# xxxupeng/stereo_toolbox

Hardware: AMD Instinct MI355X
Metric: stereo pairs/sec @ 540x960 D=192 (GwcNet_GC fwd+bwd) (higher is better)
Workload: dtype f32; 1 GPU; GwcNet_GC(maxdisp=192) train step: fwd+bwd+allreduce+Adam, 576x960 pairs (reference pad_to_2x shape), batch 1/GPU, fp32, synthetic randn inputs, deterministic filler weights; global_batch=1, parallelism=dp1, grad_sync=none (single rank: flat fp32 buffer packed, no collective), launch=eager, optimizer=torch.optim.Adam(fused=True)

## Files before the change

include/stx_hip.h:

```cpp
#ifndef STX_HIP_H
#define STX_HIP_H
#ifdef __cplusplus
extern "C" {
#endif

const char* stx_last_error(void);
const char* stx_build_info(void);
int stx_get_tuning(const char* name);
int stx_set_tuning(const char* name, int value);

int stx_cost_volume_fwd(const float* Lg, const float* Rg, int Cg, int G, const float* Lc, const float* Rc, int Cc,
                        const float* scale, float* vol, int B, int H, int W, int D, int mask_left, void* stream);
int stx_group_normalize_fwd(const float* x, float* y, int B, int C, int G, int HW, float out_scale, void* stream);
int stx_group_normalize_bwd(const float* x, const float* gy, float* gx, int B, int C, int G, int HW, float out_scale, void* stream);
int stx_cost_volume_bwd(const float* gvol, const float* Lg, const float* Rg, int Cg, int G, int Cc, float* gLg,
                        float* gRg, float* gLc, float* gRc, int B, int H, int W, int D, int mask_left, void* stream);

int stx_head_fwd(const float* cost, float* disp, float* stats, int B, int Dc, int Hc, int Wc, int D, int H, int W,
                 void* stream);
long long stx_head_bwd_workspace_floats(int B, int Dc, int H, int W);
int stx_head_bwd(const float* gdisp, const float* cost, const float* disp, const float* stats, float* gcost,
                 float* workspace, int B, int Dc, int Hc, int Wc, int D, int H, int W, void* stream);
int stx_head_fwd2(const float* cost, float* disp, float* stats, int B, int Dc, int Hc, int Wc, int D, int H, int W,
                  int align_corners, void* stream);
int stx_head_bwd2(const float* gdisp, const float* cost, const float* disp, const float* stats, float* gcost,
                  float* workspace, int B, int Dc, int Hc, int Wc, int D, int H, int W, int align_corners, void* stream);
int stx_softargmax_fwd(const float* x, float* out, int B, int D, int HW, void* stream);
int stx_argmax_fwd(const float* x, long long* out, int B, int D, int HW, void* stream);
int stx_unimodal_fwd(const float* x, float* out, int B, int D, int HW, void* stream);
int stx_dominant_modal_fwd(const float* x, float* out, int B, int D, int HW, void* stream);
int stx_modal_fwd(const float* x, float* out, float* aux, int B, int D, int HW, int kind, void* stream);
int stx_modal_bwd(const float* g, const float* out, const float* aux, float* gx, int B, int D, int HW, void* stream);
int stx_split_mode(const float* x, float* mode, unsigned char* mask, int B, int D, int HW, void* stream);
int stx_softmax_d_fwd(const float* x, float* y, int B, int D, int HW, void* stream);

long long stx_conv3d_packed_floats(int K, int N, int T);
int stx_conv3d_pack_weight(const float* w, float* wp, int A, int B, int T, int mode, void* stream);
int stx_conv3d_fwd_blocks(int Do, int Ho, int Wo);
long long stx_conv3d_fwd_stat_rows(int B, int Di, int Hi, int Wi, int Cin, int Cout, int ks, int stride);
int stx_conv3d_fwd(const float* x, const float* wp, float* out, const float* scale, const float* bias,
                   const float* residual, float* stats, int B, int Di, int Hi, int Wi, int Cin, int Cout, int ks,
                   int stride, int relu, void* stream);
int stx_deconv3d_fwd_blocks(int Di, int Hi, int Wi);
int stx_deconv3d_fwd(const float* x, const float* wp, float* out, const float* scale, const float* bias,
                     const float* residual, float* stats, int B, int Di, int Hi, int Wi, int Cin, int Cout, int Do,
                     int Ho, int Wo, int relu, void* stream);
long long stx_conv3d_wgrad_workspace_floats(int B, int Dc, int Hc, int Wc, int CF, int CC, int ks, int stride);
int stx_conv3d_wgrad(const float* fine, const float* coarse, float* dw, float* workspace, int B, int Df, int Hf, int Wf,
                     int CF, int Dc, int Hc, int Wc, int CC, int ks, int stride, void* stream);

int stx_conv3d_wgrad_bn_supported(int B, int D, int H, int W, int CF, int CC);
int stx_conv3d_wgrad_bn(const float* x, const float* gy, const float* z, const float* scale, const float* shift, const float* mean,
                        const float* invstd, const float* gamma, const float* sums, float inv_n, int act, float* dz, float* dw,
                        float* workspace, int B, int D, int H, int W, int CF, int CC, void* stream);

int stx_conv2d_supported(int Cin, int Cout);
long long stx_conv2d_stat_rows(int groups);
int stx_conv2d_fwd(const float* x, const float* w, float* out, float* stats, int B, int H, int W, int Cin, int Cout, int dgrad,
                   int groups, void* stream);

int stx_conv3d_c1_fwd(const float* x, const float* w, const float* residual, float* out, int B, int D, int H, int W,
                      int Cin, void* stream);
long long stx_conv3d_c1_wgrad_workspace_floats(int Cin);
int stx_conv3d_c1_wgrad(const float* x, const float* gy, float* dw, float* workspace, int B, int D, int H, int W,
                        int Cin, void* stream);
int stx_conv3d_c1_dgrad(const float* gy, const float* w, float* gx, int B, int D, int H, int W, int Cin, void* stream);

int stx_mish_fwd(const float* x, float* y, long long n, void* stream);
int stx_mish_bwd(const float* gy, const float* x, float* gx, long long n, void* stream);
int stx_depth_to_space(const float* y, float* out, int B, int D, int H, int W, int C, int inverse, void* stream);
int stx_gate_fwd(const float* cv, const float* att, float* out, int B, int D, long long HW, int C, void* stream);
int stx_gate_bwd(const float* g, const float* cv, const float* att, float* gcv, float* gatt, int B, int D, long long HW,
                 int C, void* stream);

int stx_concat_channels(const float* in0, const float* in1, const float* in2, const float* in3, int C0, int C1, int C2, int C3,
                        float* out, long long nvox, void* stream);
int stx_split_channels(const float* in, float* out0, float* out1, float* out2, float* out3, int C0, int C1, int C2, int C3,
                       long long nvox, void* stream);
int stx_transpose(const float* in, float* out, int N, int rows, int cols, void* stream);

int stx_dwconv_hw_fwd(const float* x, const float* w, const int* dil, float* out, int B, int D, int H, int W, int C,
                      int flip, void* stream);
long long stx_dwconv_hw_wgrad_workspace_floats(int C);
int stx_dwconv_hw_wgrad(const float* x, const float* gy, const int* dil, float* dw, float* workspace, int B, int D,
                        int H, int W, int C, void* stream);
int stx_cost_volume_scale_bwd(const float* gvol, const float* Lc, const float* Rc, float* gscale, int B, int Cc, int H,
                              int W, int D, int mask_left, void* stream);
int stx_scale_channels(const float* x, const float* s, float* out, long long nvox, int C, void* stream);
int stx_ac_volume_bwd(const float* gvol, const float* Lc, const float* Rc, const float* prob, float* gL, float* gR,
                      float* gprob, int B, int Cc, int H, int W, int D, int mask_left, void* stream);

int stx_bn_reduce_blocks(void);
int stx_bn_stats_rows(long long nvox, int C);
int stx_bn_stats(const float* z, float* partials, long long nvox, int C, int groups, void* stream);
int stx_bn_finalize(const float* partials, int nrows, int C, double count, const float* gamma, const float* beta,
                    float* running_mean, float* running_var, float momentum, float eps, float* scale, float* shift,
                    float* mean, float* invstd, void* stream);
int stx_bn_finalize_groups(const float* partials, int nrows, int C, double count, const float* gamma, const float* beta,
                           float* running_mean, float* running_var, float momentum, float eps, float* out, int groups,
                           void* stream);
int stx_bn_apply(const float* z1, const float* scale1, const float* shift1, const float* z2, const float* scale2,
                 const float* shift2, float* out, long long nvox, int C, int relu, int groups, void* stream);
int stx_bn_bwd_reduce(const float* gy, const float* y, const float* z1, const float* mean1, const float* invstd1,
                      const float* z2, const float* mean2, const float* invstd2, float* partials, float* sums,
                      long long nvox, int C, int relu, void* stream);
int stx_bn_bwd_apply(const float* gy, const float* y, const float* z1, const float* mean1, const float* invstd1,
                     const float* gamma1, const float* z2, const float* mean2, const float* invstd2,
                     const float* gamma2, const float* sums, float* dz1, float* dz2, float* gout, long long nvox, int C,
                     int relu, void* stream);
int stx_bn_bwd_reduce2(const float* gy, const float* y, const float* z1, const float* mean1, const float* invstd1,
                       const float* z2, const float* mean2, const float* invstd2, const float* scale1,
                       const float* shift1, const float* scale2, const float* shift2, float* partials, float* sums,
                       long long nvox, int C, int relu, int groups, void* stream);
int stx_bn_bwd_apply2(const float* gy, const float* y, const float* z1, const float* mean1, const float* invstd1,
                      const float* gamma1, const float* z2, const float* mean2, const float* invstd2,
                      const float* gamma2, const float* scale1, const float* shift1, const float* scale2,
                      const float* shift2, const float* sums, float* dz1, float* dz2, float* gout, long long nvox,
                      int C, int relu, int groups, void* stream);

int stx_pad_normalize_u8(const unsigned char* img, float* out, int B, int H, int W, int Hp, int Wp, int top,
                         const float* mean3, const float* std3, void* stream);

int stx_sampled_volume_fwd(const float* Lg, const float* Rg, int Cg, int G, const float* Lc, const float* Rc, int Cc,
                           const float* samples, float* vol, int B, int H, int W, int S, int CTp, void* stream);
int stx_sampled_volume_bwd(const float* gvol, const float* Lg, const float* Rg, int Cg, int G, int Cc,
                           const float* samples, float* gLg, float* gRg, float* gLc, float* gRc, int B, int H, int W,
                           int S, int CTp, void* stream);

int stx_warp_fwd(const float* x, const float* disp, float* out, int B, int C, int H, int W, void* stream);
int stx_warp_bwd(const float* gout, const float* x, const float* disp, float* gx, float* gdisp, int B, int C, int H, int W,
                 void* stream);
int stx_corr_volume_fwd(const float* ref, const float* tgt, float* vol, int B, int C, int H, int W, int maxdisp, int groups,
                        void* stream);
int stx_corr_volume_bwd(const float* gvol, const float* ref, const float* tgt, float* gref, float* gtgt, int B, int C, int H,
                        int W, int maxdisp, int groups, void* stream);
int stx_disparity_variance_fwd(const float* x, const float* disp, const float* samples, float* out, int B, int D, int HW,
                               void* stream);
int stx_disparity_variance_bwd(const float* g, const float* x, const float* disp, const float* samples, float* gx, float* gdisp,
                               float* gsamples, int B, int D, int HW, void* stream);

long long stx_geo_pyramid_floats(long long rows, int len, int C, int levels);
int stx_geo_corr_fwd(const float* fmap1, const float* fmap2, float* cpyr, int B, int C, int H, int W1, int W2, int levels,
                     void* stream);
int stx_geo_corr_bwd(const float* gcpyr, const float* fmap1, const float* fmap2, float* gfmap1, float* gfmap2, int B, int C, int H,
                     int W1, int W2, int levels, void* stream);
int stx_geo_pyramid_fwd(const float* vol, float* gpyr, int B, int D, int H, int W, int C, int levels, void* stream);
int stx_geo_pyramid_bwd(const float* ggpyr, float* gvol, int B, int D, int H, int W, int C, int levels, void* stream);
int stx_geo_lookup_fwd(const float* gpyr, const float* cpyr, const float* disp, const float* coords, float* out, int B, int H,
                       int W, int D, int C, int W2, int levels, int radius, void* stream);
int stx_geo_lookup_bwd(const float* gout, const float* disp, const float* coords, float* ggpyr, float* gcpyr, int B, int H, int W,
                       int D, int C, int W2, int levels, int radius, void* stream);
int stx_context_upsample_fwd(const float* disp_low, const float* up_weights, float* out, int B, int h, int w, void* stream);
int stx_context_upsample_bwd(const float* g, const float* disp_low, const float* up_weights, float* gdisp, float* gweights, int B,
                             int h, int w, void* stream);

long long stx_corr1d_pyramid_floats(long long rows, int W2, int levels);
int stx_corr1d_pyramid_fwd(const float* fmap1, const float* fmap2, float* cpyr, int B, int C, int H, int W1, int W2, int levels,
                           float scale, void* stream);
int stx_corr1d_pyramid_bwd(const float* gcpyr, const float* fmap1, const float* fmap2, float* gfmap1, float* gfmap2, int B, int C,
                           int H, int W1, int W2, int levels, float scale, void* stream);
int stx_corr1d_lookup_fwd(const float* cpyr, const float* base, const float* disp, const float* jobs, int njobs, float* out, int B,
                          int H, int W1, int W2, int levels, void* stream);
int stx_corr1d_lookup_bwd(const float* gout, const float* base, const float* disp, const float* jobs, int njobs, float* gcpyr,
                          int B, int H, int W1, int W2, int levels, void* stream);

int stx_allpairs_estimates_fwd(const float* vol, int which, float* disp_l, float* conf_l, float* disp_r, float* conf_r, float* stats,
                               int B, int H, int W1, int W2, void* stream);
int stx_allpairs_estimates_bwd(const float* g_disp_l, const float* g_conf_l, const float* g_disp_r, const float* g_conf_r,
                               const float* vol, const float* stats, float* gvol, int B, int H, int W1, int W2, void* stream);
int stx_corr1d_volume_pyramid_fwd(const float* vol, const float* tdisp, const float* tconf, float atten, float* cpyr, int B, int H,
                                  int W1, int W2, int levels, void* stream);
int stx_corr1d_volume_pyramid_bwd(const float* gcpyr, const float* tdisp, const float* tconf, float atten, float* gvol, int B, int H,
                                  int W1, int W2, int levels, void* stream);
int stx_truncate_mask_fwd(const float* disp, const float* conf, int has_th, float conf_th, float atten, float* mask, int B, int H,
                          int W, void* stream);

int stx_photo_warp_fwd(const float* right, const float* disp, float* warped, float* valid, int B, int C, int H, int W, void* stream);
int stx_photo_warp_bwd(const float* gwarped, const float* right, const float* disp, float* gdisp, int B, int C, int H, int W,
                       void* stream);
int stx_ssim_fwd(const float* x, const float* y, float* out, int B, int C, int H, int W, int window, void* stream);
long long stx_ssim_bwd_workspace_floats(int B, int C, int H, int W);
int stx_ssim_bwd(const float* g_out, const float* x, const float* y, float* gx, float* gy, float* workspace, int B, int C, int H, int W,
                 int window, void* stream);
int stx_photometric_fwd(const float* left, const float* right, const float* disp, double ssim_weight, int enable_mask, float* loss,
                        int B, int C, int H, int W, void* stream);
long long stx_photometric_bwd_workspace_floats(int B, int C, int H, int W);
int stx_photometric_bwd(const float* gloss, const float* left, const float* right, const float* disp, double ssim_weight,
                        int enable_mask, float* gdisp, float* workspace, int B, int C, int H, int W, void* stream);
int stx_auto_mask_fwd(const float* left, const float* right, const float* disp, int denorm, unsigned char* mask, int B, int C, int H,
                      int W, void* stream);
long long stx_smoothness_workspace_floats(int B, int H, int W);
int stx_smoothness_fwd(const float* disp, const float* img, float* out, float* stats, float* workspace, int B, int C, int H, int W,
                       void* stream);
int stx_smoothness_bwd(const float* gout, const float* disp, const float* img, const float* stats, float* gdisp, int B, int C, int H,
                       int W, void* stream);

int stx_sttr_head_fwd(const float* attn, const float* phi, int mode, int iters, float log_one, float log_bin, float log_2w,
                      const unsigned char* occ_mask, const float* target, float* disp, float* occ, float* norm, int* arg,
                      float* gt_response, float* bin_left, float* bin_right, double* us, double* vs, int N, int H, int W, void* stream);
int stx_sttr_head_bwd(const float* g_disp, const float* g_occ, const float* g_gt, const float* g_bin_left, const float* g_bin_right,
                      const float* attn, const float* phi, int mode, int iters, float log_one, float log_bin, float log_2w,
                      const float* target, const float* disp, const float* norm, const int* arg, const double* us, const double* vs,
                      float* g_attn, double* phi_partials, float* g_phi, int N, int H, int W, void* stream);
int stx_sttr_transport_fwd(const float* attn, const float* phi, int mode, int iters, float log_one, float log_bin, float log_2w,
                           float* P, double* us, double* vs, int N, int H, int W, void* stream);
int stx_sttr_transport_bwd(const float* G, const float* attn, const float* phi, int mode, int iters, float log_one, float log_bin,
                           float log_2w, const double* us, const double* vs, float* g_attn, double* phi_partials, float* g_phi, int N,
                           int H, int W, void* stream);

int stx_sttr_attn_fwd(const float* q, const float* k, const float* v, const float* Qr, const float* Kr, int causal, float* o,
                      float* raw, float* avg, float* stats, int W, int B, int E, int head_dim, void* stream);
int stx_sttr_attn_bwd(const float* dO, const float* dRaw, const float* q, const float* k, const float* v, const float* Qr,
                      const float* Kr, const float* o, const float* stats, int causal, float* dq, float* dk, float* dv, float* dQr,
                      float* dKr, float* scratch, long long scratch_floats, int nb, int W, int B, int E, int head_dim, void* stream);

int stx_convex_upsample_fwd(const float* flow, const float* mask, float* out, int N, int D, int H, int W, int mask_channels, int f,
                            float scale, void* stream);
long long stx_convex_upsample_bwd_workspace_floats(int N, int D, int H, int W);
int stx_convex_upsample_bwd(const float* g, const float* flow, const float* mask, float* gflow, float* gmask, float* workspace, int N,
                            int D, int H, int W, int mask_channels, int f, float scale, void* stream);
int stx_softmax_context_upsample_fwd(const float* disp_low, const float* logits, float* out, int B, int h, int w, float scale,
                                     void* stream);
int stx_softmax_context_upsample_bwd(const float* g, const float* disp_low, const float* logits, float* gdisp, float* glogits,
                                     float* workspace, int B, int h, int w, float scale, void* stream);
int stx_sequence_loss_max_predictions(void);
long long stx_sequence_loss_workspace_floats(long long n);
int stx_sequence_loss_fwd(const float* const* preds, const double* weights, int K, const float* gt, float maxdisp, float* loss,
                          int* count, float* workspace, long long n, void* stream);
int stx_sequence_loss_bwd(const float* gloss, const float* const* preds, const double* weights, int K, const float* gt, float maxdisp,
                          const int* count, float* const* gpreds, long long n, void* stream);

#ifdef __cplusplus
}
#endif
#endif
```

stereo_toolbox_amd/_capi.py:

```python
import ctypes
import os
import threading

import torch

_P = ctypes.c_void_p
_I = ctypes.c_int
_F = ctypes.c_float
_L = ctypes.c_longlong

SIGNATURES = {
    "stx_get_tuning": [ctypes.c_char_p],
    "stx_set_tuning": [ctypes.c_char_p, _I],
    "stx_cost_volume_fwd": [_P, _P, _I, _I, _P, _P, _I, _P, _P, _I, _I, _I, _I, _I, _P],
    "stx_cost_volume_bwd": [_P, _P, _P, _I, _I, _I, _P, _P, _P, _P, _I, _I, _I, _I, _I, _P],
    "stx_group_normalize_fwd": [_P, _P, _I, _I, _I, _I, _F, _P],
    "stx_group_normalize_bwd": [_P, _P, _P, _I, _I, _I, _I, _F, _P],
    "stx_head_fwd": [_P, _P, _P, _I, _I, _I, _I, _I, _I, _I, _P],
    "stx_head_bwd_workspace_floats": [_I, _I, _I, _I],
    "stx_head_bwd": [_P, _P, _P, _P, _P, _P, _I, _I, _I, _I, _I, _I, _I, _P],
    "stx_head_fwd2": [_P, _P, _P, _I, _I, _I, _I, _I, _I, _I, _I, _P],
    "stx_head_bwd2": [_P, _P, _P, _P, _P, _P, _I, _I, _I, _I, _I, _I, _I, _I, _P],
    "stx_softargmax_fwd": [_P, _P, _I, _I, _I, _P],
    "stx_argmax_fwd": [_P, _P, _I, _I, _I, _P],
    "stx_softmax_d_fwd": [_P, _P, _I, _I, _I, _P],
    "stx_unimodal_fwd": [_P, _P, _I, _I, _I, _P],
    "stx_dominant_modal_fwd": [_P, _P, _I, _I, _I, _P],
    "stx_modal_fwd": [_P, _P, _P, _I, _I, _I, _I, _P],
    "stx_modal_bwd": [_P, _P, _P, _P, _I, _I, _I, _P],
    "stx_split_mode": [_P, _P, _P, _I, _I, _I, _P],
    "stx_conv3d_packed_floats": [_I, _I, _I],
    "stx_conv3d_pack_weight": [_P, _P, _I, _I, _I, _I, _P],
    "stx_conv3d_fwd_blocks": [_I, _I, _I],
    "stx_conv3d_fwd_stat_rows": [_I, _I, _I, _I, _I, _I, _I, _I],
    "stx_deconv3d_fwd_blocks": [_I, _I, _I],
    "stx_conv3d_fwd": [_P, _P, _P, _P, _P, _P, _P, _I, _I, _I, _I, _I, _I, _I, _I, _I, _P],
    "stx_deconv3d_fwd": [_P, _P, _P, _P, _P, _P, _P, _I, _I, _I, _I, _I, _I, _I, _I, _I, _I, _P],
    "stx_conv3d_wgrad_workspace_floats": [_I, _I, _I, _I, _I, _I, _I, _I],
    "stx_conv3d_wgrad": [_P, _P, _P, _P, _I, _I, _I, _I, _I, _I, _I, _I, _I, _I, _I, _P],
    "stx_conv3d_wgrad_bn_supported": [_I, _I, _I, _I, _I, _I],
    "stx_conv3d_wgrad_bn": [_P] * 9 + [_F, _I, _P, _P, _P, _I, _I, _I, _I, _I, _I, _P],
    "stx_conv2d_supported": [_I, _I],
    "stx_conv2d_stat_rows": [_I],
    "stx_conv2d_fwd": [_P, _P, _P, _P, _I, _I, _I, _I, _I, _I, _I, _P],
    "stx_conv3d_c1_fwd": [_P, _P, _P, _P, _I, _I, _I, _I, _I, _P],
    "stx_conv3d_c1_wgrad_workspace_floats": [_I],
    "stx_conv3d_c1_wgrad": [_P, _P, _P, _P, _I, _I, _I, _I, _I, _P],
    "stx_conv3d_c1_dgrad": [_P, _P, _P, _I, _I, _I, _I, _I, _P],
    "stx_mish_fwd": [_P, _P, _L, _P],
    "stx_mish_bwd": [_P, _P, _P, _L, _P],
    "stx_depth_to_space": [_P, _P, _I, _I, _I, _I, _I, _I, _P],
    "stx_gate_fwd": [_P, _P, _P, _I, _I, _L, _I, _P],
    "stx_gate_bwd": [_P, _P, _P, _P, _P, _I, _I, _L, _I, _P],
    "stx_concat_channels": [_P, _P, _P, _P, _I, _I, _I, _I, _P, _L, _P],
    "stx_split_channels": [_P, _P, _P, _P, _P, _I, _I, _I, _I, _L, _P],
    "stx_transpose": [_P, _P, _I, _I, _I, _P],
    "stx_dwconv_hw_fwd": [_P, _P, _P, _P, _I, _I, _I, _I, _I, _I, _P],
    "stx_dwconv_hw_wgrad_workspace_floats": [_I],
    "stx_dwconv_hw_wgrad": [_P, _P, _P, _P, _P, _I, _I, _I, _I, _I, _P],
    "stx_cost_volume_scale_bwd": [_P, _P, _P, _P, _I, _I, _I, _I, _I, _I, _P],
    "stx_scale_channels": [_P, _P, _P, _L, _I, _P],
    "stx_ac_volume_bwd": [_P, _P, _P, _P, _P, _P, _P, _I, _I, _I, _I, _I, _I, _P],
    "stx_pad_normalize_u8": [_P, _P, _I, _I, _I, _I, _I, _I, _P, _P, _P],
    "stx_warp_fwd": [_P, _P, _P, _I, _I, _I, _I, _P],
    "stx_warp_bwd": [_P, _P, _P, _P, _P, _I, _I, _I, _I, _P],
    "stx_corr_volume_fwd": [_P, _P, _P, _I, _I, _I, _I, _I, _I, _P],
    "stx_corr_volume_bwd": [_P, _P, _P, _P, _P, _I, _I, _I, _I, _I, _I, _P],
    "stx_disparity_variance_fwd": [_P, _P, _P, _P, _I, _I, _I, _P],
    "stx_disparity_variance_bwd": [_P, _P, _P, _P, _P, _P, _P, _I, _I, _I, _P],
    "stx_sampled_volume_fwd": [_P, _P, _I, _I, _P, _P, _I, _P, _P, _I, _I, _I, _I, _I, _P],
    "stx_sampled_volume_bwd": [_P, _P, _P, _I, _I, _I, _P, _P, _P, _P, _P, _I, _I, _I, _I, _I, _P],
    "stx_geo_pyramid_floats": [_L, _I, _I, _I],
    "stx_geo_corr_fwd": [_P, _P, _P, _I, _I, _I, _I, _I, _I, _P],
    "stx_geo_corr_bwd": [_P, _P, _P, _P, _P, _I, _I, _I, _I, _I, _I, _P],
    "stx_geo_pyramid_fwd": [_P, _P, _I, _I, _I, _I, _I, _I, _P],
    "stx_geo_pyramid_bwd": [_P, _P, _I, _I, _I, _I, _I, _I, _P],
    "stx_geo_lookup_fwd": [_P, _P, _P, _P, _P, _I, _I, _I, _I, _I, _I, _I, _I, _P],
    "stx_geo_lookup_bwd": [_P, _P, _P, _P, _P, _I, _I, _I, _I, _I, _I, _I, _I, _P],
    "stx_context_upsample_fwd": [_P, _P, _P, _I, _I, _I, _P],
    "stx_context_upsample_bwd": [_P, _P, _P, _P, _P, _I, _I, _I, _P],
    "stx_corr1d_pyramid_floats": [_L, _I, _I],
    "stx_corr1d_pyramid_fwd": [_P, _P, _P, _I, _I, _I, _I, _I, _I, _F, _P],
    "stx_corr1d_pyramid_bwd": [_P, _P, _P, _P, _P, _I, _I, _I, _I, _I, _I, _F, _P],
    "stx_corr1d_lookup_fwd": [_P, _P, _P, _P, _I, _P, _I, _I, _I, _I, _I, _P],
    "stx_corr1d_lookup_bwd": [_P, _P, _P, _P, _I, _P, _I, _I, _I, _I, _I, _P],
    "stx_allpairs_estimates_fwd": [_P, _I, _P, _P, _P, _P, _P, _I, _I, _I, _I, _P],
    "stx_allpairs_estimates_bwd": [_P, _P, _P, _P, _P, _P, _P, _I, _I, _I, _I, _P],
    "stx_corr1d_volume_pyramid_fwd": [_P, _P, _P, _F, _P, _I, _I, _I, _I, _I, _P],
    "stx_corr1d_volume_pyramid_bwd": [_P, _P, _P, _F, _P, _I, _I, _I, _I, _I, _P],
    "stx_truncate_mask_fwd": [_P, _P, _I, _F, _F, _P, _I, _I, _I, _P],
    "stx_photo_warp_fwd": [_P, _P, _P, _P, _I, _I, _I, _I, _P],
    "stx_photo_warp_bwd": [_P, _P, _P, _P, _I, _I, _I, _I, _P],
    "stx_ssim_fwd": [_P, _P, _P, _I, _I, _I, _I, _I, _P],
    "stx_ssim_bwd_workspace_floats": [_I, _I, _I, _I],
    "stx_ssim_bwd": [_P, _P, _P, _P, _P, _P, _I, _I, _I, _I, _I, _P],
    "stx_photometric_fwd": [_P, _P, _P, ctypes.c_double, _I, _P, _I, _I, _I, _I, _P],
    "stx_photometric_bwd_workspace_floats": [_I, _I, _I, _I],
    "stx_photometric_bwd": [_P, _P, _P, _P, ctypes.c_double, _I, _P, _P, _I, _I, _I, _I, _P],
    "stx_auto_mask_fwd": [_P, _P, _P, _I, _P, _I, _I, _I, _I, _P],
    "stx_smoothness_workspace_floats": [_I, _I, _I],
    "stx_smoothness_fwd": [_P, _P, _P, _P, _P, _I, _I, _I, _I, _P],
    "stx_smoothness_bwd": [_P, _P, _P, _P, _P, _I, _I, _I, _I, _P],
    "stx_sttr_head_fwd": [_P, _P, _I, _I, _F, _F, _F] + [_P] * 11 + [_I, _I, _I, _P],
    "stx_sttr_head_bwd": [_P] * 7 + [_I, _I, _F, _F, _F] + [_P] * 9 + [_I, _I, _I, _P],
    "stx_sttr_transport_fwd": [_P, _P, _I, _I, _F, _F, _F, _P, _P, _P, _I, _I, _I, _P],
    "stx_sttr_transport_bwd": [_P, _P, _P, _I, _I, _F, _F, _F, _P, _P, _P, _P, _P, _I, _I, _I, _P],
    "stx_sttr_attn_fwd": [_P] * 5 + [_I] + [_P] * 4 + [_I, _I, _I, _I, _P],
    "stx_sttr_attn_bwd": [_P] * 9 + [_I] + [_P] * 6 + [_L, _I, _I, _I, _I, _I, _P],
    "stx_convex_upsample_fwd": [_P, _P, _P, _I, _I, _I, _I, _I, _I, _F, _P],
    "stx_convex_upsample_bwd_workspace_floats": [_I, _I, _I, _I],
    "stx_convex_upsample_bwd": [_P, _P, _P, _P, _P, _P, _I, _I, _I, _I, _I, _I, _F, _P],
    "stx_softmax_context_upsample_fwd": [_P, _P, _P, _I, _I, _I, _F, _P],
    "stx_softmax_context_upsample_bwd": [_P, _P, _P, _P, _P, _P, _I, _I, _I, _F, _P],
    "stx_sequence_loss_max_predictions": [],
    "stx_sequence_loss_workspace_floats": [_L],
    "stx_sequence_loss_fwd": [_P, _P, _I, _P, _F, _P, _P, _P, _L, _P],
    "stx_sequence_loss_bwd": [_P, _P, _P, _I, _P, _F, _P, _P, _L, _P],
    "stx_bn_reduce_blocks": [],
    "stx_bn_stats_rows": [_L, _I],
    "stx_bn_stats": [_P, _P, _L, _I, _I, _P],
    "stx_bn_finalize": [_P, _I, _I, ctypes.c_double, _P, _P, _P, _P, _F, _F, _P, _P, _P, _P, _P],
    "stx_bn_finalize_groups": [_P, _I, _I, ctypes.c_double, _P, _P, _P, _P, _F, _F, _P, _I, _P],
    "stx_bn_apply": [_P, _P, _P, _P, _P, _P, _P, _L, _I, _I, _I, _P],
    "stx_bn_bwd_reduce": [_P, _P, _P, _P, _P, _P, _P, _P, _P, _P, _L, _I, _I, _P],
    "stx_bn_bwd_apply": [_P, _P, _P, _P, _P, _P, _P, _P, _P, _P, _P, _P, _P, _P, _L, _I, _I, _P],
    "stx_bn_bwd_reduce2": [_P] * 14 + [_L, _I, _I, _I, _P],
    "stx_bn_bwd_apply2": [_P] * 18 + [_L, _I, _I, _I, _P],
}
_RET_CHARP = ("stx_last_error", "stx_build_info")


class StxError(RuntimeError):
    pass


class StxLib:

    def __init__(self, path):
        if not os.path.exists(path):
            raise StxError(
                f"HIP library not found: {path}. Build it with `python -m stereo_toolbox_amd.build` "
                "(hipcc, gfx950). There is no CPU fallback for the cost-volume hot path.")
        self.path = path
        self._dll = ctypes.CDLL(path)
        for name in _RET_CHARP:
            fn = getattr(self._dll, name)
            fn.restype = ctypes.c_char_p
            fn.argtypes = []
        self._fns = {}
        for name, argtypes in SIGNATURES.items():
            fn = getattr(self._dll, name, None)
            if fn is None:
                continue
            fn.restype = ctypes.c_longlong if name.endswith(("_floats", "_stat_rows")) else _I
            fn.argtypes = argtypes
            self._fns[name] = fn

    def has(self, name):
        return name in self._fns

    def build_info(self):
        return self._dll.stx_build_info().decode()

    def get_tuning(self, name):
        return self._fns["stx_get_tuning"](name.encode())

    def set_tuning(self, name, value):
        old = self.get_tuning(name)
        if old < 0 or self._fns["stx_set_tuning"](name.encode(), int(value)) != 0:
            raise StxError(f"unknown tuning switch {name}")
        return old

    def raw(self, name):
        return self._fns[name]

    def call(self, name, *args):
        fn = self._fns.get(name)
        if fn is None:
            raise StxError(f"{self.path} does not export {name}")
        rc = fn(*args)
        if rc != 0:
            raise StxError(f"{name} failed ({rc}): {self._dll.stx_last_error().decode()}")


_LIB = None
_LOCK = threading.Lock()
LIB_PATH = os.environ.get("STX_HIP_LIB") or os.path.join(os.path.dirname(os.path.abspath(__file__)), "lib", "libstx_hip.so")


def get_lib():
    global _LIB
    if _LIB is None:
        with _LOCK:
            if _LIB is None:
                _LIB = StxLib(LIB_PATH)
    return _LIB
```

stereo_toolbox_amd/aggregation.py:

```python
import os
import threading

import torch
import torch.nn as nn

from . import ops


def _is_transposed(conv):
    return isinstance(conv, nn.ConvTranspose3d)


def _conv_cfg(conv):
    ks = conv.kernel_size[0]
    stride = conv.stride[0]
    if _is_transposed(conv):
        k3 = ks == 3 and stride == 2 and conv.padding[0] == 1 and conv.output_padding[0] == 1
        k4 = ks == 4 and stride == 2 and conv.padding[0] == 1 and conv.output_padding[0] == 0
        if not (k3 or k4) or len(set(conv.kernel_size)) != 1 or len(set(conv.stride)) != 1:
            raise ops.StxError("only ConvTranspose3d(k=3, s=2, p=1, op=1) and ConvTranspose3d(k=4, s=2, p=1) are on the hot path")
    else:
        if not ((ks == 3 and conv.padding[0] == 1 and stride in (1, 2)) or (ks == 1 and conv.padding[0] == 0 and stride == 1)):
            raise ops.StxError(f"unsupported Conv3d k={ks} s={stride} p={conv.padding}")
    if conv.bias is not None or conv.groups != 1:
        raise ops.StxError("hot-path convolutions are bias-free and dense")
    return ks, stride


def _fold(bn):
    key = (bn.weight._version, bn.bias._version, bn.running_mean._version, bn.running_var._version,
           bn.weight.data_ptr(), bn.bias.data_ptr(), bn.running_mean.data_ptr(), bn.running_var.data_ptr())
    hit = bn.__dict__.get("_stx_fold") if ops._CACHE_ENABLED else None
    if hit is not None and hit[0] == key:
        return hit[1], hit[2]
    with torch.no_grad():
        scale = (bn.weight * torch.rsqrt(bn.running_var + bn.eps)).contiguous()
        bias = (bn.bias - bn.running_mean * scale).contiguous()
    if ops._CACHE_ENABLED:
        bn.__dict__["_stx_fold"] = (key, scale, bias)
    return scale, bias


def _needs_grad(*tensors_and_modules):
    if not torch.is_grad_enabled():
        return False
    for t in tensors_and_modules:
        if t is None:
            continue
        if isinstance(t, torch.Tensor):
            if t.requires_grad:
                return True
        else:
            if any(p.requires_grad for p in t.parameters()):
                return True
    return False


def _infer_conv(x, conv, scale, bias, residual, relu):
    ks, stride = _conv_cfg(conv)
    if _is_transposed(conv) and ks == 4:
        if residual is not None:
            raise ops.StxError("ConvTranspose3d(k4) with a fused residual is not wired (no model uses it)")
        return ops.deconv4_forward(x, conv.weight.detach(), scale, bias, int(relu), owner=conv.weight)
    if _is_transposed(conv):
        wp = ops.pack_weight(conv.weight.detach(), 2, owner=conv.weight)
        return ops.deconv3d_forward(x, wp, conv.weight.shape[1], scale=scale, bias=bias, residual=residual, relu=relu)[0]
    if ops._is_c1(conv.weight, ks, stride, False) and scale is None and bias is None and not relu:
        return ops.conv3d_c1_forward(x, conv.weight.detach().contiguous(), residual)
    if x.shape[-1] != conv.weight.shape[1]:
        if x.shape[-1] != (conv.weight.shape[1] + 7) // 8 * 8:
            raise ops.StxError(f"conv: input has {x.shape[-1]} channels, weight expects {conv.weight.shape[1]}")
        wpad = ops.pad_weight_channels(conv.weight.detach(), x.shape[-1])
        return ops.conv3d_forward(x, ops.pack_weight(wpad, 0), conv.weight.shape[0], ks, stride, scale, bias, residual, relu)[0]
    if x.shape[-1] % 8 != 0:
        xp, wpad = ops.pad_input_channels(x, conv.weight.detach())
        return ops.conv3d_forward(xp, ops.pack_weight(wpad, 0), conv.weight.shape[0], ks, stride, scale, bias, residual, relu)[0]
    wp = ops.pack_weight(conv.weight.detach(), 0, owner=conv.weight)
    return ops.conv3d_forward(x, wp, conv.weight.shape[0], ks, stride, scale, bias, residual, relu)[0]


class deferred_bn_counters:
    _tls = threading.local()

    @staticmethod
    def _state():
        st = deferred_bn_counters._tls
        if not hasattr(st, "active"):
            st.active, st.pending = 0, []
        return st

    def __enter__(self):
        self._state().active += 1
        ops.bn_defer_reset_if_stale()
        return self

    def __exit__(self, *exc):
        st = self._state()
        st.active -= 1
        if st.active == 0 and st.pending:
            pend, st.pending = st.pending, []
            by_dev = {}
            for t in pend:
                d = by_dev.setdefault(t.device, {})
                ent = d.setdefault(id(t), [t, 0])
                ent[1] += 1
            for d in by_dev.values():
                torch._foreach_add_([e[0] for e in d.values()], [e[1] for e in d.values()])
        return False


def _bn_state(bn, partials, count, steps=1):
    training = bn.training
    sync = None
    if training and isinstance(bn, nn.SyncBatchNorm):
        import torch.distributed as dist
        if dist.is_available() and dist.is_initialized() and dist.get_world_size(bn.process_group) > 1:
            sync = (bn.process_group, dist.get_world_size(bn.process_group))
    if training:
        bn.__dict__.pop("_stx_fold", None)
    if training and bn.track_running_stats and bn.num_batches_tracked is not None:
        st = deferred_bn_counters._state()
        if st.active and bn.momentum is not None:
            st.pending.extend([bn.num_batches_tracked] * steps)
        else:
            bn.num_batches_tracked.add_(steps)
    if bn.momentum is not None:
        momentum = bn.momentum
    elif training and bn.track_running_stats and bn.num_batches_tracked is not None:
        momentum = 1.0 / float(bn.num_batches_tracked.item())
    else:
        momentum = 0.0
    return {"training": training, "partials": partials, "count": count, "running_mean": bn.running_mean,
            "running_var": bn.running_var, "momentum": momentum, "eps": bn.eps, "sync": sync}


def _raw_conv(x, conv, want):
    ks, stride = _conv_cfg(conv)
    if _is_transposed(conv) and ks == 4:
        return ops.deconv4_raw(x, conv.weight, want)
    return ops.ConvRawFn.apply(x, conv.weight, ks, stride, _is_transposed(conv), want)


@ops.fp32_region
def shared_input_convs(x, blocks):
    cfgs, ws = [], []
    for seq in blocks:
        conv, bn = seq[0], seq[1]
        if _is_transposed(conv) or not bn.training or conv.weight.shape[1] != x.shape[-1] or conv.weight.shape[1] % 8 \
                or conv.weight.shape[0] % 8:
            return None
        ks, stride = _conv_cfg(conv)
        cfgs.append((ks, stride, True))
        ws.append(conv.weight)
    if not _needs_grad(x, *[m for seq in blocks for m in (seq[0], seq[1])]):
        return None
    outs = ops.SharedInputConvsFn.apply(x, tuple(cfgs), *ws)
    return [(outs[2 * k], outs[2 * k + 1]) for k in range(len(blocks))]


@ops.fp32_region
def conv_block(x, conv, bn=None, relu=False, second=None, residual=None, mish=False, leaky=False, raw=None, second_raw=None):
    if (mish and relu) or (leaky and (relu or mish)):
        raise ops.StxError("conv_block: relu, mish and leaky are mutually exclusive")
    if second is not None and residual is not None:
        raise ops.StxError("conv_block: `second` and `residual` are mutually exclusive")
    mods = [conv, bn] + ([second[1], second[2]] if second is not None else [])
    grad = (raw is not None or second_raw is not None
            or _needs_grad(x, residual, *(m for m in mods if m is not None), *([second[0]] if second else [])))
    train_bn = (bn is not None and bn.training) or (second is not None and second[2].training)
    if mish and (grad or train_bn) and (bn is None or residual is not None):
        return ops.mish(conv_block(x, conv, bn, relu=False, second=second, residual=residual))
    if mish:
        relu = 2
    if leaky:
        relu = 3

    if not grad and not train_bn:
        if second is not None:
            s2, b2 = _fold(second[2])
            residual = _infer_conv(second[0], second[1], s2, b2, None, False)
        if bn is not None:
            s1, b1 = _fold(bn)
        else:
            s1 = b1 = None
        return _infer_conv(x, conv, s1, b1, residual, relu)

    want = bn is not None and bn.training
    z1, part1 = raw if raw is not None else _raw_conv(x, conv, want)
    if bn is None:
        y = z1
        if residual is not None:
            y = y + residual
        if relu == 3:
            return torch.nn.functional.leaky_relu(y, 0.01)
        return torch.relu(y) if relu else y
    count1 = z1.numel() // z1.shape[-1]
    st1 = _bn_state(bn, part1 if want else None, count1)
    if second is not None:
        x2, conv2, bn2 = second
        want2 = bn2.training
        z2, part2 = second_raw if second_raw is not None else _raw_conv(x2, conv2, want2)
        st2 = _bn_state(bn2, part2 if want2 else None, z2.numel() // z2.shape[-1])
        return ops.BnActFn.apply(z1, bn.weight, bn.bias, z2, bn2.weight, bn2.bias, None, relu, st1, st2)
    defer = (residual is None and want and relu in (0, 1, False, True) and not _is_transposed(conv) and _conv_cfg(conv) == (3, 1)
             and conv.weight.shape[0] % 32 == 0 and conv.weight.shape[1] % 32 == 0 and not st1.get("sync")
             and os.environ.get("STX_BN_BWD_IN_WGRAD", "1") != "0")
    if defer:
        ops.bn_defer_reset_if_stale()
    return ops.BnActFn.apply(z1, bn.weight, bn.bias, None, None, None, residual, relu, st1, None, 1, defer)


@ops.fp32_region
def convbn_block(x, seq, relu=False, second=None, residual=None, mish=False, raw=None, second_raw=None):
    sec = None
    if second is not None:
        sec = (second[0], second[1][0], second[1][1])
    return conv_block(x, seq[0], seq[1], relu=relu, second=sec, residual=residual, mish=mish, raw=raw, second_raw=second_raw)
```

stereo_toolbox_amd/csrc/conv2d.hip:

```cpp
#include "stx_common.h"

namespace {

constexpr int C2_THREADS = 256;
constexpr int C2_TH = 8, C2_TW = 16, C2_EH = C2_TH + 2, C2_EW = C2_TW + 2, C2_NV = C2_EH * C2_EW;

struct Conv2dArgs {
    const float* x;
    const float* w;
    float* out;
    float* stats;
    int B, H, W, Cin, Cout;
    int nHt, nWt, groups;
    int dgrad;
};

__device__ __forceinline__ f32x4 c2_zero4() { f32x4 z = {0.f, 0.f, 0.f, 0.f}; return z; }

template <int KQ, int ABL = 0, int PAD = 8>
__global__ __launch_bounds__(C2_THREADS) void conv2d_march_kernel(Conv2dArgs a) {
    constexpr int CIN = 16 * KQ, VS = CIN + PAD, F4 = CIN / 4;
    constexpr int WFLOATS = 9 * KQ * 256;
    constexpr int NST = (C2_NV * F4 + C2_THREADS - 1) / C2_THREADS;
    constexpr int SLOT = (NST * C2_THREADS / F4) * VS;
    constexpr int NSTEP = 9 * KQ;
    STX_DYN_SMEM(smem);
    float* wl = reinterpret_cast<float*>(smem);
    float* bufs = wl + WFLOATS;
    float* ssum = bufs + 2 * SLOT;

    const int tid = threadIdx.x, lane = tid & 63, wave = __builtin_amdgcn_readfirstlane(tid >> 6);
    const int i = lane & 15, kg = lane >> 4;

    const int wgs_g = gridDim.x / a.groups;
    const int grp = blockIdx.x / wgs_g, wl_id = blockIdx.x - grp * wgs_g;
    const int tiles_img = a.nHt * a.nWt;
    const int tiles_g = (a.B / a.groups) * tiles_img;
    const int nsl = a.Cout / 16;
    const long long units = (long long)tiles_g * nsl;
    const bool idle = grp >= a.groups;
    int u = idle ? 0 : __builtin_amdgcn_readfirstlane((int)(units * wl_id / wgs_g));
    const int u_end = idle ? 0 : __builtin_amdgcn_readfirstlane((int)(units * (wl_id + 1) / wgs_g));

    if (a.stats) {
        for (int e = tid; e < 2 * a.Cout; e += C2_THREADS) ssum[e] = 0.f;
    }

    unsigned rel[NST];
    int crd[NST];
#pragma unroll
    for (int k = 0; k < NST; ++k) {
        const int e = tid + k * C2_THREADS;
        const int v = e / F4, f = e - v * F4;
        const int hy = v / C2_EW, wx = v - hy * C2_EW;
        crd[k] = e < C2_NV * F4 ? (hy << 8 | wx) : -1;
        rel[k] = (unsigned)(((hy * a.W + wx) * CIN + 4 * f) * 4);
    }
    float4 stg[NST];
    auto decode = [&](int uu, int& slice, int& b, int& oh0, int& ow0) {
        slice = uu / tiles_g;
        const int t = uu - slice * tiles_g;
        const int bl = t / tiles_img, r = t - bl * tiles_img;
        const int ht = r / a.nWt, wt = r - ht * a.nWt;
        b = grp * (a.B / a.groups) + bl;
        oh0 = ht * C2_TH; ow0 = wt * C2_TW;
    };
    auto load_tile = [&](int b, int oh0, int ow0) {
        const long long org = (long long)(oh0 - 1) * a.W + (ow0 - 1), img = (long long)a.H * a.W;
        const stx_bufrsrc rs = stx_make_rsrc(a.x + ((long long)b * img + org) * CIN, (unsigned)((img - org) * CIN * 4));
#pragma unroll
        for (int k = 0; k < NST; ++k) {
            const int gh = oh0 - 1 + (crd[k] >> 8), gw = ow0 - 1 + (crd[k] & 255);
            const bool ok = crd[k] >= 0 && gh >= 0 && gh < a.H && gw >= 0 && gw < a.W;
            stg[k] = stx_buf_ld4(rs, ok ? rel[k] : STX_BUF_OOB, 0u);
        }
    };
    auto store_tile = [&](float* buf) {
#pragma unroll
        for (int k = 0; k < NST; ++k) {
            const int e = tid + k * C2_THREADS;
            const int v = e / F4, f = e - v * F4;
            if (e < C2_NV * F4) stx_st4(buf + v * VS + 4 * f, stg[k]);
        }
    };
    auto load_weights = [&](int slice) {
        if (!a.dgrad) {
            for (int e = tid; e < WFLOATS / 4; e += C2_THREADS) {
                const int l = e & 63, ts = e >> 6, tap = ts / KQ, s = ts - tap * KQ;
                stx_st4(wl + 4 * e, stx_ld4(a.w + ((size_t)(16 * slice + (l & 15)) * 9 + tap) * CIN + 16 * s + 4 * (l >> 4)));
            }
        } else {
            for (int e = tid; e < CIN * 9 * 4; e += C2_THREADS) {
                const int q = e & 3, kt = e >> 2, tap = kt % 9, k = kt / 9;
                const float4 v = stx_ld4(a.w + ((size_t)k * 9 + (8 - tap)) * a.Cout + 16 * slice + 4 * q);
                float* dst = wl + ((tap * KQ + (k >> 4)) * 64 + 4 * q + 16 * ((k & 15) >> 2)) * 4 + (k & 3);
                dst[0] = v.x; dst[4] = v.y; dst[8] = v.z; dst[12] = v.w;
            }
        }
    };

    f32x4 pacc0 = c2_zero4(), pacc1 = c2_zero4();
    unsigned pvoff[2] = {STX_BUF_OOB, STX_BUF_OOB}, cvoff[2] = {STX_BUF_OOB, STX_BUF_OOB};
    stx_bufrsrc prs = stx_make_rsrc(a.out, 0u);
    float s1[4] = {0.f, 0.f, 0.f, 0.f}, s2[4] = {0.f, 0.f, 0.f, 0.f};
    auto emit_prev = [&](int r) {
        f32x4 v = r ? pacc1 : pacc0;
        const bool ok = (int)pvoff[r] >= 0;
#pragma unroll
        for (int c = 0; c < 4; ++c) {
            v[c] = ok ? v[c] : 0.f;
            s1[c] += v[c];
            s2[c] = fmaf(v[c], v[c], s2[c]);
        }
        stx_buf_st4(prs, pvoff[r], 0u, make_float4(v[0], v[1], v[2], v[3]));
    };
    auto flush_stats = [&](int slice) {
#pragma unroll
        for (int c = 0; c < 4; ++c) {
#pragma unroll
            for (int d = 1; d < 16; d <<= 1) { s1[c] += __shfl_xor(s1[c], d); s2[c] += __shfl_xor(s2[c], d); }
        }
        for (int w = 0; w < 4; ++w) {
            if (wave == w && i == 0) {
#pragma unroll
                for (int c = 0; c < 4; ++c) {
                    ssum[16 * slice + 4 * kg + c] += s1[c];
                    ssum[a.Cout + 16 * slice + 4 * kg + c] += s2[c];
                }
            }
            __syncthreads();
        }
#pragma unroll
        for (int c = 0; c < 4; ++c) { s1[c] = 0.f; s2[c] = 0.f; }
    };

    const int abase0 = ((2 * wave) * C2_EW + i) * VS + 4 * kg, abase1 = abase0 + C2_EW * VS;
    const float* wlane = wl + lane * 4;

    int slice = 0, b = 0, oh0 = 0, ow0 = 0;
    if (u < u_end) {
        decode(u, slice, b, oh0, ow0);
        load_weights(slice);
        load_tile(b, oh0, ow0);
        store_tile(bufs);
    }
    __syncthreads();
    int cur = 0;
    while (u < u_end) {
        const bool more = u + 1 < u_end;
        int nslice = slice, nb = b, noh0 = oh0, now0 = ow0;
        if (more) decode(u + 1, nslice, nb, noh0, now0);
        const long long norg = (long long)(noh0 - 1) * a.W + (now0 - 1), img = (long long)a.H * a.W;
        const stx_bufrsrc nrs = stx_make_rsrc(a.x + ((long long)nb * img + norg) * CIN, more ? (unsigned)((img - norg) * CIN * 4) : 0u);
        const stx_bufrsrc crs = stx_make_rsrc(a.out + (size_t)b * img * a.Cout, (unsigned)(img * a.Cout * 4));
        const float* pbuf = bufs + cur * SLOT;
        float* nbuf = bufs + (cur ^ 1) * SLOT;
        f32x4 acc0, acc1;
        float4 av0[3], av1[3], bv[3];
        auto load_step = [&](int st, int slot) {
            const int tap = st / KQ, s = st - tap * KQ;
            const int kh = tap / 3, kw = tap - 3 * kh;
            const float* sl = pbuf + (kh * C2_EW + kw) * VS + 16 * s;
            av0[slot] = stx_ld4(sl + abase0);
            av1[slot] = stx_ld4(sl + abase1);
            bv[slot] = stx_ld4(wlane + st * 256);
        };
        load_step(0, 0);
        load_step(1, 1);
#pragma unroll
        for (int st = 0; st < NSTEP; ++st) {
            if (st + 2 < NSTEP) load_step(st + 2, (st + 2) % 3);
            const int cb = st % 3;
            acc0 = __builtin_amdgcn_mfma_f32_16x16x4f32(bv[cb].x, av0[cb].x, st == 0 ? c2_zero4() : acc0, 0, 0, 0);
            acc1 = __builtin_amdgcn_mfma_f32_16x16x4f32(bv[cb].x, av1[cb].x, st == 0 ? c2_zero4() : acc1, 0, 0, 0);
            acc0 = __builtin_amdgcn_mfma_f32_16x16x4f32(bv[cb].y, av0[cb].y, acc0, 0, 0, 0);
            acc1 = __builtin_amdgcn_mfma_f32_16x16x4f32(bv[cb].y, av1[cb].y, acc1, 0, 0, 0);
            acc0 = __builtin_amdgcn_mfma_f32_16x16x4f32(bv[cb].z, av0[cb].z, acc0, 0, 0, 0);
            acc1 = __builtin_amdgcn_mfma_f32_16x16x4f32(bv[cb].z, av1[cb].z, acc1, 0, 0, 0);
            acc0 = __builtin_amdgcn_mfma_f32_16x16x4f32(bv[cb].w, av0[cb].w, acc0, 0, 0, 0);
            acc1 = __builtin_amdgcn_mfma_f32_16x16x4f32(bv[cb].w, av1[cb].w, acc1, 0, 0, 0);
            if (st < NST) {
                const unsigned gh = (unsigned)(noh0 - 1 + (crd[st] >> 8)), gw = (unsigned)(now0 - 1 + (crd[st] & 255));
                const bool ok = (crd[st] >= 0) & (gh < (unsigned)a.H) & (gw < (unsigned)a.W);
                if (!(ABL & 1)) stg[st] = stx_buf_ld4(nrs, ok ? rel[st] : STX_BUF_OOB, 0u);
            }
            if ((st == 0 || st == 4) && !(ABL & 4)) emit_prev(st >> 2);
            if (st == 8 || st == 9) {
                const int r = st - 8;
                const int oh = oh0 + 2 * wave + r, ow = ow0 + i;
                cvoff[r] = (unsigned)((((oh * a.W + ow) * a.Cout) + 16 * slice + 4 * kg) * 4) | (((oh < a.H) & (ow < a.W)) ? 0u : STX_BUF_OOB);
            }
            if (st >= NSTEP - NST) {
                const int k = st - (NSTEP - NST);
                const int e = tid + k * C2_THREADS;
                const int v = e / F4, f = e - v * F4;
                if (!(ABL & 2)) stx_st4(nbuf + v * VS + 4 * f, stg[k]);
            }
            STX_SCHED_GROUP(0x008, 1); STX_SCHED_GROUP(0x100, 1);
            STX_SCHED_GROUP(0x008, 1); STX_SCHED_GROUP(0x100, 1);
            STX_SCHED_GROUP(0x008, 1); STX_SCHED_GROUP(0x100, 1);
            STX_SCHED_GROUP(0x008, 1); STX_SCHED_GROUP(0x002, 4);
            STX_SCHED_GROUP(0x008, 1); STX_SCHED_GROUP(0x010, 1); STX_SCHED_GROUP(0x002, 4);
            STX_SCHED_GROUP(0x008, 1); STX_SCHED_GROUP(0x010, 1); STX_SCHED_GROUP(0x002, 4);
            STX_SCHED_GROUP(0x008, 1); STX_SCHED_GROUP(0x200, 1); STX_SCHED_GROUP(0x002, 4);
            STX_SCHED_GROUP(0x008, 1);
            STX_SCHED_BARRIER();
        }
        prs = crs;
        pvoff[0] = cvoff[0]; pvoff[1] = cvoff[1];
        pacc0 = acc0; pacc1 = acc1;
        if (!(ABL & 8)) __syncthreads();
        if (more && nslice != slice) {
            emit_prev(0); emit_prev(1);
            pvoff[0] = pvoff[1] = STX_BUF_OOB;
            if (a.stats) flush_stats(slice);
            load_weights(nslice);
            __syncthreads();
        }
        slice = nslice; b = nb; oh0 = noh0; ow0 = now0;
        cur ^= 1;
        ++u;
    }
    emit_prev(0); emit_prev(1);
    if (a.stats) {
        __syncthreads();
        if (u_end > 0 && !idle) flush_stats(slice);
        __syncthreads();
        for (int e = tid; e < 2 * a.Cout; e += C2_THREADS) a.stats[(size_t)blockIdx.x * 2 * a.Cout + e] = ssum[e];
    }
}

int conv2d_grid(int groups) {
    int g = 256;
    g -= g % groups;
    return g < groups ? groups : g;
}

}

extern "C" int stx_conv2d_supported(int Cin, int Cout) {
    stx_begin();
    return (Cin == 32 || Cin == 64) && Cout >= 16 && Cout % 16 == 0 && Cout <= 256;
}

extern "C" long long stx_conv2d_stat_rows(int groups) {
    stx_begin();
    return groups >= 1 && groups <= 256 ? conv2d_grid(groups) : 0;
}

extern "C" int stx_conv2d_fwd(const float* x, const float* w, float* out, float* stats, int B, int H, int W, int Cin, int Cout,
                              int dgrad, int groups, void* stream) {
    stx_begin();
    STX_REQUIRE(x && w && out && B > 0 && H > 0 && W > 0 && (dgrad == 0 || dgrad == 1), "conv2d_fwd: bad args");
    STX_REQUIRE(stx_conv2d_supported(Cin, Cout), "conv2d_fwd: %d -> %d channels unsupported (Cin 32 or 64, Cout a multiple of 16)", Cin, Cout);
    STX_REQUIRE(groups >= 1 && groups <= 256 && B % groups == 0, "conv2d_fwd: batch %d does not split into %d groups", B, groups);
    STX_REQUIRE((long long)(H + 2) * W * (Cin > Cout ? Cin : Cout) * 4 < (1ll << 31), "conv2d_fwd: image too large for one descriptor");
    STX_REQUIRE(H < 32768 && W < 32768, "conv2d_fwd: image too large");
    Conv2dArgs a;
    a.x = x; a.w = w; a.out = out; a.stats = stats; a.dgrad = dgrad;
    a.B = B; a.H = H; a.W = W; a.Cin = Cin; a.Cout = Cout;
    a.nHt = stx_cdiv(H, C2_TH); a.nWt = stx_cdiv(W, C2_TW); a.groups = groups;
    const int grid = conv2d_grid(groups);
    int pad = stx_tune(STX_TUNE_C2_PAD);
    if (pad != 4 && pad != 12) pad = 8;
    const size_t lds = ((size_t)9 * Cin * 16 + (size_t)2 * 192 * (Cin + pad) + (size_t)2 * Cout) * 4;
    void (*k)(Conv2dArgs) = Cin == 64 ? conv2d_march_kernel<4> : conv2d_march_kernel<2>;
    if (pad == 4) k = Cin == 64 ? conv2d_march_kernel<4, 0, 4> : conv2d_march_kernel<2, 0, 4>;
    if (pad == 12) k = Cin == 64 ? conv2d_march_kernel<4, 0, 12> : conv2d_march_kernel<2, 0, 12>;
    const int abl = stx_tune(STX_TUNE_C2_ABLATE);
    if (abl && Cin == 64 && pad == 8)
        k = abl == 1 ? conv2d_march_kernel<4, 1> : abl == 2 ? conv2d_march_kernel<4, 2> : abl == 3 ? conv2d_march_kernel<4, 3>
          : abl == 4 ? conv2d_march_kernel<4, 4> : abl == 7 ? conv2d_march_kernel<4, 7> : abl == 8 ? conv2d_march_kernel<4, 8>
          : conv2d_march_kernel<4, 15>;
    if (int rc = stx_lds_require((const void*)k, lds, "conv2d_fwd")) return rc;
    hipLaunchKernelGGL(k, dim3(grid), dim3(C2_THREADS), lds, (hipStream_t)stream, a);
    return stx_check_launch("conv2d_fwd");
}
```

stereo_toolbox_amd/models/ACVNet/acv.py:

```python
import torch
import torch.nn as nn

from ... import ops
from ...aggregation import convbn_block, deferred_bn_counters, shared_input_convs
from ..features2d import ResTrunk, cat_features, channels_last_weights_, convbn, init_reference_style, run_head2d, run_pair
from ..GwcNet.gwcnet import classifier, run_classifier
from .submodule import attention_block, convbn_3d


class feature_extraction(ResTrunk):
    fused_everywhere = True

    def forward(self, x):
        return {"gwc_feature": cat_features(self.trunk(x))}


class hourglass(nn.Module):

    def __init__(self, c):
        super().__init__()
        self.conv1 = nn.Sequential(convbn_3d(c, c * 2, 3, 2, 1), nn.ReLU(inplace=True))
        self.conv2 = nn.Sequential(convbn_3d(c * 2, c * 2, 3, 1, 1), nn.ReLU(inplace=True))
        self.conv3 = nn.Sequential(convbn_3d(c * 2, c * 4, 3, 2, 1), nn.ReLU(inplace=True))
        self.conv4 = nn.Sequential(convbn_3d(c * 4, c * 4, 3, 1, 1), nn.ReLU(inplace=True))
        self.attention_block = attention_block(channels_3d=c * 4, num_heads=16, block=(4, 4, 4))
        self.conv5 = nn.Sequential(nn.ConvTranspose3d(c * 4, c * 2, 3, padding=1, output_padding=1, stride=2, bias=False),
                                   nn.BatchNorm3d(c * 2))
        self.conv6 = nn.Sequential(nn.ConvTranspose3d(c * 2, c, 3, padding=1, output_padding=1, stride=2, bias=False),
                                   nn.BatchNorm3d(c))
        self.redir1 = convbn_3d(c, c, kernel_size=1, stride=1, pad=0)
        self.redir2 = convbn_3d(c * 2, c * 2, kernel_size=1, stride=1, pad=0)

    def forward(self, x):
        rx = shared_input_convs(x, [self.conv1[0], self.redir1]) or [None, None]
        c1 = convbn_block(x, self.conv1[0], relu=True, raw=rx[0])
        c2 = convbn_block(c1, self.conv2[0], relu=True)
        r2 = shared_input_convs(c2, [self.conv3[0], self.redir2]) or [None, None]
        c3 = convbn_block(c2, self.conv3[0], relu=True, raw=r2[0])
        c4 = convbn_block(c3, self.conv4[0], relu=True)
        c4 = self.attention_block(c4)
        c5 = convbn_block(c4, self.conv5, relu=True, second=(c2, self.redir2), second_raw=r2[1])
        return convbn_block(c5, self.conv6, relu=True, second=(x, self.redir1), second_raw=rx[1])


class ACVNet(nn.Module):
    def __init__(self, maxdisp=192, attn_weights_only=False, freeze_attn_weights=False):
        super().__init__()
        self.maxdisp = maxdisp
        self.attn_weights_only = attn_weights_only
        self.freeze_attn_weights = freeze_attn_weights
        self.num_groups = 40
        self.concat_channels = 32
        self.feature_extraction = feature_extraction()
        self.concatconv = nn.Sequential(convbn(320, 128, 3, 1, 1, 1), nn.ReLU(inplace=True),
                                        nn.Conv2d(128, self.concat_channels, kernel_size=1, padding=0, stride=1, bias=False))
        self.patch = nn.Conv3d(40, 40, kernel_size=(1, 3, 3), stride=1, dilation=1, groups=40, padding=(0, 1, 1), bias=False)
        self.patch_l1 = nn.Conv3d(8, 8, kernel_size=(1, 3, 3), stride=1, dilation=1, groups=8, padding=(0, 1, 1), bias=False)
        self.patch_l2 = nn.Conv3d(16, 16, kernel_size=(1, 3, 3), stride=1, dilation=2, groups=16, padding=(0, 2, 2), bias=False)
        self.patch_l3 = nn.Conv3d(16, 16, kernel_size=(1, 3, 3), stride=1, dilation=3, groups=16, padding=(0, 3, 3), bias=False)
        self.dres1_att_ = nn.Sequential(convbn_3d(40, 32, 3, 1, 1), nn.ReLU(inplace=True), convbn_3d(32, 32, 3, 1, 1))
        self.dres2_att_ = hourglass(32)
        self.classif_att_ = classifier(32)
        self.dres0 = nn.Sequential(convbn_3d(self.concat_channels * 2, 32, 3, 1, 1), nn.ReLU(inplace=True),
                                   convbn_3d(32, 32, 3, 1, 1), nn.ReLU(inplace=True))
        self.dres1 = nn.Sequential(convbn_3d(32, 32, 3, 1, 1), nn.ReLU(inplace=True), convbn_3d(32, 32, 3, 1, 1))
        self.dres2 = hourglass(32)
        self.dres3 = hourglass(32)
        self.classif0 = classifier(32)
        self.classif1 = classifier(32)
        self.classif2 = classifier(32)
        init_reference_style(self)
        channels_last_weights_(self.feature_extraction)
        channels_last_weights_(self.concatconv)
        self._dil = {}

    def _dilations(self, device):
        key = str(device)
        if key not in self._dil:
            one = torch.ones(10, dtype=torch.int32, device=device)
            two = torch.tensor([1] * 2 + [2] * 4 + [3] * 4, dtype=torch.int32, device=device)
            self._dil[key] = (one, two)
        return self._dil[key]

    def _attention_branch(self, gl, gr):
        gwc = ops.cost_volume(gl, gr, None, None, self.maxdisp // 4, self.num_groups)
        d1, d2 = self._dilations(gwc.device)
        v = ops.dwconv_hw(gwc, self.patch.weight.reshape(40, 9), d1)
        w2 = torch.cat((self.patch_l1.weight.reshape(8, 9), self.patch_l2.weight.reshape(16, 9),
                        self.patch_l3.weight.reshape(16, 9)), 0)
        pv = ops.dwconv_hw(v, w2, d2)
        t = convbn_block(pv, self.dres1_att_[0], relu=True)
        ca = convbn_block(t, self.dres1_att_[2], relu=False)
        ca = self.dres2_att_(ca)
        return run_classifier(self.classif_att_, ca)

    def forward(self, left, right):
        with deferred_bn_counters():
            H, W = left.shape[2], left.shape[3]
            if self.freeze_attn_weights:
                with torch.no_grad():
                    fl, fr = run_pair(self.feature_extraction, left, right, self.training)
            else:
                fl, fr = run_pair(self.feature_extraction, left, right, self.training)
            return self._aggregate(fl["gwc_feature"], fr["gwc_feature"], H, W)

    def aggregate(self, gl, gr, H, W, concat_left=None, concat_right=None):
        with deferred_bn_counters():
            return self._aggregate(gl, gr, H, W, concat_left, concat_right)

    @ops.fp32_region
    def _aggregate(self, gl, gr, H, W, cl=None, cr=None):
        if self.freeze_attn_weights:
            with torch.no_grad():
                att = self._attention_branch(gl, gr)
        else:
            att = self._attention_branch(gl, gr)

        if not self.attn_weights_only:
            if cl is None:
                cl, cr = run_head2d(self.concatconv, gl), run_head2d(self.concatconv, gr)
            if torch.is_grad_enabled() and att.requires_grad:
                prob = torch.softmax(att, dim=1)
            else:
                prob = ops.softmax_over_d(att.contiguous())
            ac = ops.ac_volume(cl, cr, prob, self.maxdisp // 4)
            cost0 = convbn_block(ac, self.dres0[0], relu=True)
            cost0 = convbn_block(cost0, self.dres0[2], relu=True)
            t = convbn_block(cost0, self.dres1[0], relu=True)
            cost0 = convbn_block(t, self.dres1[2], relu=False, residual=cost0)
            out1 = self.dres2(cost0)
            out2 = self.dres3(out1)

        if self.training:
            preds = []
            if not self.freeze_attn_weights:
                preds.append(ops.regression_head(att, self.maxdisp, H, W))
            if not self.attn_weights_only:
                preds += [ops.regression_head(run_classifier(c, o), self.maxdisp, H, W)
                          for c, o in ((self.classif0, cost0), (self.classif1, out1), (self.classif2, out2))]
            return preds
        if self.attn_weights_only:
            return ops.regression_head(att, self.maxdisp, H, W)
        return ops.regression_head(run_classifier(self.classif2, out2), self.maxdisp, H, W)
```

stereo_toolbox_amd/models/GwcNet/gwcnet.py:

```python
import torch
import torch.nn as nn

from ... import ops
from ...aggregation import conv_block, convbn_block, deferred_bn_counters, shared_input_convs
from ..features2d import ResTrunk, cat_features, channels_last_weights_, convbn, init_reference_style, run_head2d, run_pair
from .submodule import convbn_3d


class feature_extraction(ResTrunk):
    fused_everywhere = True

    def __init__(self, concat_feature=False, concat_feature_channel=12):
        super().__init__()
        self.concat_feature = concat_feature
        if concat_feature:
            self.lastconv = nn.Sequential(convbn(320, 128, 3, 1, 1, 1), nn.ReLU(inplace=True),
                                          nn.Conv2d(128, concat_feature_channel, 1, bias=False))

    def forward(self, x):
        gwc = cat_features(self.trunk(x))
        if not self.concat_feature:
            return {"gwc_feature": gwc}
        return {"gwc_feature": gwc, "concat_feature": run_head2d(self.lastconv, gwc)}


class hourglass(nn.Module):

    def __init__(self, c):
        super().__init__()
        self.conv1 = nn.Sequential(convbn_3d(c, c * 2, 3, 2, 1), nn.ReLU(inplace=True))
        self.conv2 = nn.Sequential(convbn_3d(c * 2, c * 2, 3, 1, 1), nn.ReLU(inplace=True))
        self.conv3 = nn.Sequential(convbn_3d(c * 2, c * 4, 3, 2, 1), nn.ReLU(inplace=True))
        self.conv4 = nn.Sequential(convbn_3d(c * 4, c * 4, 3, 1, 1), nn.ReLU(inplace=True))
        self.conv5 = nn.Sequential(nn.ConvTranspose3d(c * 4, c * 2, 3, padding=1, output_padding=1, stride=2, bias=False),
                                   nn.BatchNorm3d(c * 2))
        self.conv6 = nn.Sequential(nn.ConvTranspose3d(c * 2, c, 3, padding=1, output_padding=1, stride=2, bias=False),
                                   nn.BatchNorm3d(c))
        self.redir1 = convbn_3d(c, c, kernel_size=1, stride=1, pad=0)
        self.redir2 = convbn_3d(c * 2, c * 2, kernel_size=1, stride=1, pad=0)

    def forward(self, x, mid=None, also=None):
        rx = shared_input_convs(x, [self.conv1[0], self.redir1] + ([also] if also is not None else []))
        rx = rx or [None, None, None]
        c1 = convbn_block(x, self.conv1[0], relu=True, raw=rx[0])
        c2 = convbn_block(c1, self.conv2[0], relu=True)
        r2 = shared_input_convs(c2, [self.conv3[0], self.redir2]) or [None, None]
        c3 = convbn_block(c2, self.conv3[0], relu=True, raw=r2[0])
        c4 = convbn_block(c3, self.conv4[0], relu=True)
        if mid is not None:
            c4 = mid(c4)
        c5 = convbn_block(c4, self.conv5, relu=True, second=(c2, self.redir2), second_raw=r2[1])
        out = convbn_block(c5, self.conv6, relu=True, second=(x, self.redir1), second_raw=rx[1])
        return (out, rx[2]) if also is not None else out


def classifier(c):
    return nn.Sequential(convbn_3d(c, c, 3, 1, 1), nn.ReLU(inplace=True),
                         nn.Conv3d(c, 1, kernel_size=3, padding=1, stride=1, bias=False))


def run_classifier(seq, x, add=None, raw=None):
    h = convbn_block(x, seq[0], relu=True, raw=raw)
    cost = conv_block(h, seq[2], residual=None if add is None else add.unsqueeze(-1))
    return cost.squeeze(-1)


class GwcNet(nn.Module):
    def __init__(self, maxdisp, use_concat_volume=False):
        super().__init__()
        self.maxdisp = maxdisp
        self.use_concat_volume = use_concat_volume
        self.num_groups = 40
        if use_concat_volume:
            self.concat_channels = 12
            self.feature_extraction = feature_extraction(True, self.concat_channels)
        else:
            self.concat_channels = 0
            self.feature_extraction = feature_extraction(False)
        self.dres0 = nn.Sequential(convbn_3d(self.num_groups + self.concat_channels * 2, 32, 3, 1, 1),
                                   nn.ReLU(inplace=True), convbn_3d(32, 32, 3, 1, 1), nn.ReLU(inplace=True))
        self.dres1 = nn.Sequential(convbn_3d(32, 32, 3, 1, 1), nn.ReLU(inplace=True), convbn_3d(32, 32, 3, 1, 1))
        self.dres2 = hourglass(32)
        self.dres3 = hourglass(32)
        self.dres4 = hourglass(32)
        self.classif0 = classifier(32)
        self.classif1 = classifier(32)
        self.classif2 = classifier(32)
        self.classif3 = classifier(32)
        init_reference_style(self)
        channels_last_weights_(self.feature_extraction)

    def forward(self, left, right):
        with deferred_bn_counters():
            fl, fr = run_pair(self.feature_extraction, left, right, self.training)
            return self.aggregate(fl, fr, left.shape[2], left.shape[3])

    @ops.fp32_region
    def aggregate(self, fl, fr, H, W):
        vol = ops.cost_volume(fl["gwc_feature"], fr["gwc_feature"], fl.get("concat_feature"),
                              fr.get("concat_feature"), self.maxdisp // 4, self.num_groups, mask_left=True)
        cost0 = convbn_block(vol, self.dres0[0], relu=True)
        cost0 = convbn_block(cost0, self.dres0[2], relu=True)
        t = convbn_block(cost0, self.dres1[0], relu=True)
        cost0 = convbn_block(t, self.dres1[2], relu=False, residual=cost0)
        if self.training:
            out1, r0 = self.dres2(cost0, also=self.classif0[0])
            out2, r1 = self.dres3(out1, also=self.classif1[0])
            out3, r2 = self.dres4(out2, also=self.classif2[0])
            return [ops.regression_head(run_classifier(c, o, raw=r), self.maxdisp, H, W)
                    for c, o, r in ((self.classif0, cost0, r0), (self.classif1, out1, r1), (self.classif2, out2, r2),
                                    (self.classif3, out3, None))]
        out1 = self.dres2(cost0)
        out2 = self.dres3(out1)
        out3 = self.dres4(out2)
        return ops.regression_head(run_classifier(self.classif3, out3), self.maxdisp, H, W)


def GwcNet_G(d=192):
    return GwcNet(d, use_concat_volume=False)


def GwcNet_GC(d=192):
    return GwcNet(d, use_concat_volume=True)
```

stereo_toolbox_amd/models/PSMNet/stackhourglass.py:

```python
import torch.nn as nn

from ... import ops
from ...aggregation import conv_block, convbn_block, deferred_bn_counters
from ..features2d import channels_last_weights_, init_reference_style, run_pair
from .submodule import convbn_3d, feature_extraction


class hourglass(nn.Module):

    def __init__(self, inplanes):
        super().__init__()
        c = inplanes
        self.conv1 = nn.Sequential(convbn_3d(c, c * 2, kernel_size=3, stride=2, pad=1), nn.ReLU(inplace=True))
        self.conv2 = convbn_3d(c * 2, c * 2, kernel_size=3, stride=1, pad=1)
        self.conv3 = nn.Sequential(convbn_3d(c * 2, c * 2, kernel_size=3, stride=2, pad=1), nn.ReLU(inplace=True))
        self.conv4 = nn.Sequential(convbn_3d(c * 2, c * 2, kernel_size=3, stride=1, pad=1), nn.ReLU(inplace=True))
        self.conv5 = nn.Sequential(nn.ConvTranspose3d(c * 2, c * 2, kernel_size=3, padding=1, output_padding=1,
                                                      stride=2, bias=False), nn.BatchNorm3d(c * 2))
        self.conv6 = nn.Sequential(nn.ConvTranspose3d(c * 2, c, kernel_size=3, padding=1, output_padding=1,
                                                      stride=2, bias=False), nn.BatchNorm3d(c))

    def forward(self, x, presqu, postsqu, skip=None):
        out = convbn_block(x, self.conv1[0], relu=True)
        pre = convbn_block(out, self.conv2, relu=True, residual=postsqu)
        out = convbn_block(pre, self.conv3[0], relu=True)
        out = convbn_block(out, self.conv4[0], relu=True)
        post = convbn_block(out, self.conv5, relu=True, residual=presqu if presqu is not None else pre)
        out = convbn_block(post, self.conv6, relu=False, residual=skip)
        return out, pre, post


def _classifier():
    return nn.Sequential(convbn_3d(32, 32, 3, 1, 1), nn.ReLU(inplace=True),
                         nn.Conv3d(32, 1, kernel_size=3, padding=1, stride=1, bias=False))


def _run_classifier(seq, x, add=None):
    h = convbn_block(x, seq[0], relu=True)
    cost = conv_block(h, seq[2], residual=None if add is None else add.unsqueeze(-1))
    return cost.squeeze(-1)


class PSMNet(nn.Module):
    def __init__(self, maxdisp=192):
        super().__init__()
        self.maxdisp = maxdisp
        self.feature_extraction = feature_extraction()
        self.dres0 = nn.Sequential(convbn_3d(64, 32, 3, 1, 1), nn.ReLU(inplace=True),
                                   convbn_3d(32, 32, 3, 1, 1), nn.ReLU(inplace=True))
        self.dres1 = nn.Sequential(convbn_3d(32, 32, 3, 1, 1), nn.ReLU(inplace=True), convbn_3d(32, 32, 3, 1, 1))
        self.dres2 = hourglass(32)
        self.dres3 = hourglass(32)
        self.dres4 = hourglass(32)
        self.classif1 = _classifier()
        self.classif2 = _classifier()
        self.classif3 = _classifier()
        init_reference_style(self)
        channels_last_weights_(self.feature_extraction)

    def forward(self, left, right):
        with deferred_bn_counters():
            fl, fr = run_pair(self.feature_extraction, left, right, self.training)
            return self.aggregate(fl, fr, left.shape[2], left.shape[3])

    @ops.fp32_region
    def aggregate(self, fl, fr, H, W):
        cost = ops.cost_volume(None, None, fl, fr, self.maxdisp // 4, 0, mask_left=True)
        cost0 = convbn_block(cost, self.dres0[0], relu=True)
        cost0 = convbn_block(cost0, self.dres0[2], relu=True)
        t = convbn_block(cost0, self.dres1[0], relu=True)
        cost0 = convbn_block(t, self.dres1[2], relu=False, residual=cost0)
        out1, pre1, post1 = self.dres2(cost0, None, None, skip=cost0)
        out2, pre2, post2 = self.dres3(out1, pre1, post1, skip=cost0)
        out3, pre3, post3 = self.dres4(out2, pre1, post2, skip=cost0)
        cost1 = _run_classifier(self.classif1, out1)
        cost2 = _run_classifier(self.classif2, out2, add=cost1)
        cost3 = _run_classifier(self.classif3, out3, add=cost2)
        pred3 = ops.regression_head(cost3, self.maxdisp, H, W).unsqueeze(1)
        if self.training:
            pred1 = ops.regression_head(cost1, self.maxdisp, H, W).unsqueeze(1)
            pred2 = ops.regression_head(cost2, self.maxdisp, H, W).unsqueeze(1)
            return [pred1, pred2, pred3]
        return pred3
```

stereo_toolbox_amd/models/features2d.py:

```python
import math
import os
import threading

import torch
import torch.nn as nn
import torch.nn.functional as F

from .. import ops
from ..aggregation import _bn_state, _fold


def channels_last_weights_(module):
    for m in module.modules():
        if isinstance(m, nn.Conv2d) and m.weight.dim() == 4:
            m.weight.data = m.weight.data.contiguous(memory_format=torch.channels_last)
    return module


def fused_glue(x, *bns):
    if os.environ.get("STX_FEAT2D_FUSED", "1") == "0":
        return False
    if x.dtype != torch.float32 or not ops.on_device(x):
        return False
    if ops.autocast_active():
        return False
    if not all(isinstance(b, nn.modules.batchnorm._BatchNorm) for b in bns):
        return False
    if all(b.training for b in bns):
        return True
    return (not torch.is_grad_enabled() and not any(b.training for b in bns)
            and all(b.track_running_stats and b.running_mean is not None for b in bns))


class view_groups:
    _tls = threading.local()

    def __init__(self, n):
        self.new = int(n)

    @staticmethod
    def current():
        return getattr(view_groups._tls, "n", 1)

    def __enter__(self):
        self.old, view_groups._tls.n = view_groups.current(), self.new
        return self

    def __exit__(self, *exc):
        view_groups._tls.n = self.old
        return False


def _nhwc(t):
    v = t.permute(0, 2, 3, 1)
    return v if v.is_contiguous() else v.contiguous()


def cat_features(parts):
    parts = list(parts)
    if (os.environ.get("STX_FEAT2D_FUSED", "1") != "0" and os.environ.get("STX_FEAT2D_FUSED_CAT", "1") != "0" and 2 <= len(parts) <= 4
            and all(p.dtype == torch.float32 and ops.on_device(p) and p.shape[1] % 4 == 0
                    and p.is_contiguous(memory_format=torch.channels_last) for p in parts)):
        return ops.cat_channels([_nhwc(p) for p in parts]).permute(0, 3, 1, 2)
    return torch.cat(parts, dim=1)


def own_conv2d(x, conv):
    return (os.environ.get("STX_FEAT2D_CONV", "1") != "0" and x.dtype == torch.float32 and ops.on_device(x)
            and ops.conv2d_supported(conv) and x.shape[0] % view_groups.current() == 0)


def conv_bn_act(x, conv, bn, relu=False, residual=None, second=None):
    G = view_groups.current()
    part = None
    if bn.training and own_conv2d(x, conv):
        zl, part = ops.Conv2dFn.apply(x, conv.weight, G)
        z = zl.permute(0, 3, 1, 2)
    else:
        z = F.conv2d(x, conv.weight, conv.bias, conv.stride, conv.padding, conv.dilation, conv.groups)
        zl = _nhwc(z)
    if not bn.training:
        if torch.is_grad_enabled() and (z.requires_grad or bn.weight.requires_grad):
            raise ops.StxError("conv_bn_act: eval-mode BatchNorm under autograd has no fused backward -- gate the call "
                               "with fused_glue() over every BatchNorm of the block")
        sc, sh = _fold(bn)
        if second is not None:
            sc2, sh2 = _fold(second[1])
            y = ops.bn_apply(zl, sc, sh, _nhwc(second[0]), sc2, sh2, relu)
        else:
            y = ops.bn_apply(zl, sc, sh, None if residual is None else _nhwc(residual), None, None, relu)
        return y.permute(0, 3, 1, 2)
    st = _bn_state(bn, part if part is not None else ops.bn_stats(zl.detach(), G), zl.numel() // zl.shape[-1] // G, steps=G)
    if second is not None:
        z2l = _nhwc(second[0])
        bn2 = second[1]
        st2 = _bn_state(bn2, ops.bn_stats(z2l.detach(), G), z2l.numel() // z2l.shape[-1] // G, steps=G)
        y = ops.BnActFn.apply(zl, bn.weight, bn.bias, z2l, bn2.weight, bn2.bias, None, relu, st, st2, G)
    else:
        y = ops.BnActFn.apply(zl, bn.weight, bn.bias, None, None, None, None if residual is None else _nhwc(residual),
                              relu, st, None, G)
    return y.permute(0, 3, 1, 2)


def convbn_relu_chain(seq, x):
    i, n = 0, len(seq)
    while i < n:
        m = seq[i]
        if isinstance(m, nn.Sequential) and len(m) == 2 and isinstance(m[0], nn.Conv2d):
            relu = i + 1 < n and isinstance(seq[i + 1], nn.ReLU)
            x = conv_bn_act(x, m[0], m[1], relu=relu)
            i += 2 if relu else 1
        else:
            x = m(x)
            i += 1
    return x


def _chain_bns(seq):
    return [m[1] for m in seq if isinstance(m, nn.Sequential) and len(m) == 2 and isinstance(m[0], nn.Conv2d)]


def run_head2d(seq, x):
    if fused_glue(x, *_chain_bns(seq)):
        return convbn_relu_chain(seq, x)
    return seq(x)


def convbn(cin, cout, k, stride, pad, dilation):
    return nn.Sequential(
        nn.Conv2d(cin, cout, k, stride, dilation if dilation > 1 else pad, dilation, bias=False),
        nn.BatchNorm2d(cout))


class BasicBlock(nn.Module):
    expansion = 1

    def __init__(self, inplanes, planes, stride, downsample, pad, dilation):
        super().__init__()
        self.conv1 = nn.Sequential(convbn(inplanes, planes, 3, stride, pad, dilation), nn.ReLU(inplace=True))
        self.conv2 = convbn(planes, planes, 3, 1, pad, dilation)
        self.downsample = downsample
        self.stride = stride

    def forward(self, x):
        bns = [self.conv1[0][1], self.conv2[1]] + ([self.downsample[1]] if self.downsample is not None else [])
        if fused_glue(x, *bns):
            y = conv_bn_act(x, self.conv1[0][0], self.conv1[0][1], relu=True)
            if self.downsample is None:
                return conv_bn_act(y, self.conv2[0], self.conv2[1], residual=x)
            d = self.downsample[0]
            zd = F.conv2d(x, d.weight, d.bias, d.stride, d.padding, d.dilation, d.groups)
            return conv_bn_act(y, self.conv2[0], self.conv2[1], second=(zd, self.downsample[1]))
        y = self.conv2(self.conv1(x))
        if self.downsample is not None:
            x = self.downsample(x)
        return y + x


class ResTrunk(nn.Module):

    def __init__(self):
        super().__init__()
        self.inplanes = 32
        self.firstconv = nn.Sequential(convbn(3, 32, 3, 2, 1, 1), nn.ReLU(inplace=True),
                                       convbn(32, 32, 3, 1, 1, 1), nn.ReLU(inplace=True),
                                       convbn(32, 32, 3, 1, 1, 1), nn.ReLU(inplace=True))
        self.layer1 = self._make_layer(32, 3, 1, 1, 1)
        self.layer2 = self._make_layer(64, 16, 2, 1, 1)
        self.layer3 = self._make_layer(128, 3, 1, 1, 1)
        self.layer4 = self._make_layer(128, 3, 1, 1, 2)

    def _make_layer(self, planes, blocks, stride, pad, dilation):
        down = None
        if stride != 1 or self.inplanes != planes:
            down = nn.Sequential(nn.Conv2d(self.inplanes, planes, 1, stride, bias=False), nn.BatchNorm2d(planes))
        layers = [BasicBlock(self.inplanes, planes, stride, down, pad, dilation)]
        self.inplanes = planes
        layers += [BasicBlock(planes, planes, 1, None, pad, dilation) for _ in range(1, blocks)]
        return nn.Sequential(*layers)

    def trunk(self, x):
        if fused_glue(x, *_chain_bns(self.firstconv)):
            x = convbn_relu_chain(self.firstconv, x.contiguous(memory_format=torch.channels_last))
        else:
            x = self.firstconv(x)
        x = self.layer1(x)
        l2 = self.layer2(x)
        l3 = self.layer3(l2)
        l4 = self.layer4(l3)
        return l2, l3, l4


def init_reference_style(model):
    for m in model.modules():
        if isinstance(m, (nn.Conv2d, nn.Conv3d)):
            n = m.out_channels
            for k in m.kernel_size:
                n *= k
            m.weight.data.normal_(0, math.sqrt(2.0 / n))
        elif isinstance(m, (nn.BatchNorm2d, nn.BatchNorm3d)):
            m.weight.data.fill_(1)
            m.bias.data.zero_()
        elif isinstance(m, nn.Linear):
            m.bias.data.zero_()


class _SplitViewsFn(torch.autograd.Function):

    @staticmethod
    def forward(ctx, both, B):
        ctx.B, ctx.n, ctx.fmt = B, both.shape[0], (torch.channels_last if both.dim() == 4 and
                                                   both.is_contiguous(memory_format=torch.channels_last) else torch.contiguous_format)
        return both[:B], both[B:]

    @staticmethod
    def backward(ctx, gl, gr):
        if gl is None and gr is None:
            return None, None
        ref = gl if gl is not None else gr
        if gl is None:
            gl = ref.new_zeros((ctx.B,) + tuple(ref.shape[1:]))
        if gr is None:
            gr = ref.new_zeros((ctx.n - ctx.B,) + tuple(ref.shape[1:]))
        return torch.cat((gl.contiguous(memory_format=ctx.fmt), gr.contiguous(memory_format=ctx.fmt)), 0), None


def _split_views(both, B):
    if isinstance(both, dict):
        halves = {k: _SplitViewsFn.apply(v, B) for k, v in both.items()}
        return {k: h[0] for k, h in halves.items()}, {k: h[1] for k, h in halves.items()}
    return _SplitViewsFn.apply(both, B)


def run_pair(extractor, left, right, training):
    if training:
        bns = [m for m in extractor.modules() if isinstance(m, nn.modules.batchnorm._BatchNorm)]
        if (os.environ.get("STX_FEAT2D_PAIRED", "1") != "0" and left.shape == right.shape and bns and fused_glue(left, *bns)
                and all(b.momentum is not None and not isinstance(b, nn.SyncBatchNorm) for b in bns)
                and getattr(extractor, "fused_everywhere", False)):
            with view_groups(2):
                both = extractor(torch.cat((left, right), 0))
            return _split_views(both, left.shape[0])
        return extractor(left), extractor(right)
    both = extractor(torch.cat((left, right), 0))
    B = left.shape[0]
    if isinstance(both, dict):
        return {k: v[:B] for k, v in both.items()}, {k: v[B:] for k, v in both.items()}
    return both[:B], both[B:]
```

stereo_toolbox_amd/ops.py:

```python
import ctypes

import torch

from ._capi import StxError, get_lib

_P = ctypes.c_void_p


class _DevPtr(ctypes.c_void_p):
    """A device pointer that remembers the device of the tensor it came from: _call() reads the launch device off its
    own arguments, so nothing survives between launches (an exception between building the arguments and the launch
    cannot leak state into the next one)."""


def _stream(dev=None):
    return _P(torch.cuda.current_stream(dev).cuda_stream)


def _p(t):
    if t is None:
        return None
    p = _DevPtr(t.data_ptr())
    p.dev = t.device
    return p


def on_device(t):
    return t.is_cuda


def _chk(t, name, dims=None):
    if t is None:
        return
    if not t.is_cuda:
        raise StxError(f"{name}: expected a ROCm device tensor, got {t.device} -- the cost-volume hot path has "
                       "no CPU fallback (the CPU oracle lives in oracle/ and is test-only)")
    if t.dtype != torch.float32:
        raise StxError(f"{name}: expected float32, got {t.dtype}")
    if not t.is_contiguous():
        raise StxError(f"{name}: expected a dense contiguous tensor, strides {t.stride()}")
    if dims is not None and t.dim() != dims:
        raise StxError(f"{name}: expected {dims} dims, got shape {tuple(t.shape)}")


def _call(name, *args):
    dev = None
    for a in args:
        if isinstance(a, _DevPtr):
            if dev is None:
                dev = a.dev
            elif a.dev != dev:
                raise StxError(f"{name}: operands live on different devices ({dev} and {a.dev})")
    if dev is not None and dev.type == "cuda" and dev.index != torch.cuda.current_device():
        with torch.cuda.device(dev):
            get_lib().call(name, *args, _stream(dev))
    else:
        get_lib().call(name, *args, _stream(dev))


_LOW = (torch.float16, torch.bfloat16)


def _to_fp32(v):
    if isinstance(v, torch.Tensor):
        return v.float() if v.dtype in _LOW else v
    if isinstance(v, dict):
        return {k: _to_fp32(x) for k, x in v.items()}
    if isinstance(v, (list, tuple)):
        return type(v)(_to_fp32(x) for x in v)
    return v


def autocast_active():
    return torch.is_autocast_enabled("cuda") or torch.is_autocast_enabled("cpu")


def fp32_region(fn):
    import functools

    @functools.wraps(fn)
    def wrapped(*args, **kwargs):
        if not autocast_active():
            return fn(*args, **kwargs)
        with torch.autocast("cuda", enabled=False), torch.autocast("cpu", enabled=False):
            return fn(*_to_fp32(args), **_to_fp32(kwargs))
    return wrapped


def to_ncdhw(x):
    return x.permute(0, 4, 1, 2, 3)


def to_ndhwc(x):
    return x.permute(0, 2, 3, 4, 1).contiguous()


class _Workspace:

    def __init__(self):
        self.bufs = {}

    def get(self, tag, nfloats, device):
        sid = torch.cuda.current_stream(device).cuda_stream if device.type == "cuda" else 0
        key = (device.index, sid, tag)
        b = self.bufs.get(key)
        if b is None or b.numel() < nfloats:
            b = torch.empty(int(nfloats), dtype=torch.float32, device=device)
            self.bufs[key] = b
        return b


_WS = _Workspace()


_CACHE_ENABLED = True


def set_weight_cache(enabled):
    global _CACHE_ENABLED
    _CACHE_ENABLED = bool(enabled)


def invalidate_caches(model):
    for m in model.modules():
        m.__dict__.pop("_stx_fold", None)
    for p in model.parameters():
        p.__dict__.pop("_stx_packed", None)


def pack_weight(w, mode, owner=None):
    _chk(w, "weight", 5)
    if owner is not None and _CACHE_ENABLED:
        cache = owner.__dict__.setdefault("_stx_packed", {})
        hit = cache.get(mode)
        if hit is not None and hit[0] == (owner._version, owner.data_ptr()):
            return hit[1]
    A, Bd = w.shape[0], w.shape[1]
    T = w.shape[2] * w.shape[3] * w.shape[4]
    K, N = (Bd, A) if mode == 0 else (A, Bd)
    n = get_lib().raw("stx_conv3d_packed_floats")(K, N, T)
    wp = torch.empty(n, dtype=torch.float32, device=w.device)
    _call("stx_conv3d_pack_weight", _p(w), _p(wp), A, Bd, T, mode)
    if owner is not None and _CACHE_ENABLED:
        cache[mode] = ((owner._version, owner.data_ptr()), wp)
    return wp


def _pad_channels(t, C):
    if t.shape[-1] == C:
        return t
    out = t.new_zeros(*t.shape[:-1], C)
    out[..., : t.shape[-1]] = t
    return out


def pad_input_channels(x, w):
    Cin = x.shape[-1]
    Cp = (Cin + 7) // 8 * 8
    if Cp == Cin:
        return x, w
    wp = w.new_zeros(w.shape[0], Cp, *w.shape[2:])
    wp[:, :Cin] = w
    return _pad_channels(x, Cp), wp


def pad_weight_channels(w, Cp):
    if w.shape[1] == Cp:
        return w
    wp = w.new_zeros(w.shape[0], Cp, *w.shape[2:])
    wp[:, : w.shape[1]] = w
    return wp


def conv_out_dims(D, H, W, ks, stride):
    pad = ks // 2
    return tuple((d + 2 * pad - ks) // stride + 1 for d in (D, H, W))


def conv3d_forward(x, wp, Cout, ks, stride, scale=None, bias=None, residual=None, relu=False, want_stats=False):
    _chk(x, "x", 5)
    B, D, H, W, Cin = x.shape
    Do, Ho, Wo = conv_out_dims(D, H, W, ks, stride)
    out = torch.empty(B, Do, Ho, Wo, Cout, dtype=torch.float32, device=x.device)
    stats = None
    if want_stats:
        rows = get_lib().raw("stx_conv3d_fwd_stat_rows")(B, D, H, W, Cin, Cout, ks, stride)
        stats = torch.empty(rows, 2, Cout, dtype=torch.float32, device=x.device)
    _call("stx_conv3d_fwd", _p(x), _p(wp), _p(out), _p(scale), _p(bias), _p(residual), _p(stats), B, D, H, W, Cin,
          Cout, ks, stride, int(relu))
    return out, stats


def deconv3d_forward(x, wp, Cout, out_dims=None, scale=None, bias=None, residual=None, relu=False, want_stats=False):
    _chk(x, "x", 5)
    B, D, H, W, Cin = x.shape
    Do, Ho, Wo = out_dims if out_dims is not None else (2 * D, 2 * H, 2 * W)
    if Cout > 64:
        if Cout % 64 != 0:
            raise StxError(f"deconv3d_forward: Cout={Cout} > 64 must be a multiple of 64")
        nt = Cout // 32
        wv = wp.view(-1, Cin // 8, nt, 256)
        outs, sts = [], []
        for h in range(Cout // 64):
            sl = slice(64 * h, 64 * h + 64)
            o, st_ = deconv3d_forward(x, wv[:, :, 2 * h:2 * h + 2].contiguous(), 64, (Do, Ho, Wo),
                                      None if scale is None else scale[sl].contiguous(),
                                      None if bias is None else bias[sl].contiguous(),
                                      None if residual is None else residual[..., sl].contiguous(), relu, want_stats)
            outs.append(o)
            sts.append(st_)
        return torch.cat(outs, -1), (torch.cat(sts, -1) if want_stats else None)
    out = torch.empty(B, Do, Ho, Wo, Cout, dtype=torch.float32, device=x.device)
    stats = None
    if want_stats:
        nb = get_lib().raw("stx_deconv3d_fwd_blocks")(D, H, W)
        stats = torch.empty(B * nb, 2, Cout, dtype=torch.float32, device=x.device)
    _call("stx_deconv3d_fwd", _p(x), _p(wp), _p(out), _p(scale), _p(bias), _p(residual), _p(stats), B, D, H, W, Cin,
          Cout, Do, Ho, Wo, int(relu))
    return out, stats


def conv3d_wgrad(fine, coarse, ks, stride):
    B, Df, Hf, Wf, CF = fine.shape
    _, Dc, Hc, Wc, CC = coarse.shape
    n = get_lib().raw("stx_conv3d_wgrad_workspace_floats")(B, Dc, Hc, Wc, CF, CC, ks, stride)
    ws = _WS.get("wgrad", n, fine.device)
    dw = torch.empty(CC, CF, ks ** 3, dtype=torch.float32, device=fine.device)
    _call("stx_conv3d_wgrad", _p(fine), _p(coarse), _p(dw), _p(ws), B, Df, Hf, Wf, CF, Dc, Hc, Wc, CC, ks, stride)
    return dw


def conv3d_wgrad_bn(x, gy, pend):
    B, D, H, W, CF = x.shape
    CC = gy.shape[-1]
    n = get_lib().raw("stx_conv3d_wgrad_workspace_floats")(B, D, H, W, CF, CC, 3, 1)
    ws = _WS.get("wgrad", n, x.device)
    dw = torch.empty(CC, CF, 27, dtype=torch.float32, device=x.device)
    dz = torch.empty_like(gy)
    _call("stx_conv3d_wgrad_bn", _p(x), _p(gy), _p(pend.z), _p(pend.scale), _p(pend.shift), _p(pend.mean), _p(pend.invstd),
          _p(pend.gamma), _p(pend.sums), float(pend.inv_n), int(pend.act), _p(dz), _p(dw), _p(ws), B, D, H, W, CF, CC)
    return dw, dz


class _PendingBn:
    __slots__ = ("g", "z", "scale", "shift", "mean", "invstd", "gamma", "sums", "inv_n", "act")

    def materialize(self):
        C = self.z.shape[-1]
        nvox = self.z.numel() // C
        dz = torch.empty_like(self.z)
        _call("stx_bn_bwd_apply2", _p(self.g), None, _p(self.z), _p(self.mean), _p(self.invstd), _p(self.gamma), None, None,
              None, None, _p(self.scale), _p(self.shift), None, None, _p(self.sums), _p(dz), None, None, nvox, C, int(self.act), 1)
        return dz


_BN_DEFER = {"outstanding": 0, "armed": False}


def _bn_defer_check():
    n, _BN_DEFER["outstanding"], _BN_DEFER["armed"] = _BN_DEFER["outstanding"], 0, False
    if n:
        raise StxError(f"{n} deferred BatchNorm-backward record(s) were not consumed by their convolution's backward node: "
                       "the gradients of this backward pass are wrong (set STX_BN_BWD_IN_WGRAD=0 and report)")


def _defer_pending_bn(g, pend):
    g._stx_pending_bn = pend
    _BN_DEFER["outstanding"] += 1
    if not _BN_DEFER["armed"]:
        _BN_DEFER["armed"] = True
        torch.autograd.Variable._execution_engine.queue_callback(_bn_defer_check)


def bn_defer_reset_if_stale():
    if not _BN_DEFER["armed"]:
        return
    task_id = getattr(torch._C, "_current_graph_task_id", None)
    if task_id is None or task_id() == -1:
        _BN_DEFER["outstanding"], _BN_DEFER["armed"] = 0, False


def _take_pending_bn(g):
    pend = getattr(g, "_stx_pending_bn", None) if g is not None else None
    if pend is not None:
        del g._stx_pending_bn
        _BN_DEFER["outstanding"] -= 1
        if pend.g is not g:
            raise StxError("deferred BatchNorm backward: record attached to a different gradient tensor")
    return pend


def _is_c1(w, ks, stride, transposed):
    return (not transposed) and ks == 3 and stride == 1 and w.shape[0] == 1 and w.shape[1] % 16 == 0 and w.shape[1] <= 64


def conv3d_c1_forward(x, w, residual=None):
    _chk(x, "x", 5)
    _chk(w, "weight", 5)
    B, D, H, W, Cin = x.shape
    out = torch.empty(B, D, H, W, 1, dtype=torch.float32, device=x.device)
    _call("stx_conv3d_c1_fwd", _p(x), _p(w), _p(residual), _p(out), B, D, H, W, Cin)
    return out


def conv3d_c1_wgrad(x, gy):
    B, D, H, W, Cin = x.shape
    ws = _WS.get("c1wgrad", get_lib().raw("stx_conv3d_c1_wgrad_workspace_floats")(Cin), x.device)
    dw = torch.empty(1, Cin, 3, 3, 3, dtype=torch.float32, device=x.device)
    _call("stx_conv3d_c1_wgrad", _p(x), _p(gy), _p(dw), _p(ws), B, D, H, W, Cin)
    return dw


def conv3d_c1_dgrad(gy, w, Cin):
    B, D, H, W, _ = gy.shape
    gx = torch.empty(B, D, H, W, Cin, dtype=torch.float32, device=gy.device)
    _call("stx_conv3d_c1_dgrad", _p(gy), _p(w), _p(gx), B, D, H, W, Cin)
    return gx


class ConvRawFn(torch.autograd.Function):

    @staticmethod
    def forward(ctx, x, w, ks, stride, transposed, want_stats):
        _chk(x, "x", 5)
        ctx.cin_true = None
        ctx.x_prepadded = False
        if not transposed and x.shape[-1] != w.shape[1]:
            if x.shape[-1] != (w.shape[1] + 7) // 8 * 8:
                raise StxError(f"conv: input has {x.shape[-1]} channels, weight expects {w.shape[1]}")
            ctx.cin_true, ctx.x_prepadded = w.shape[1], True
            w = pad_weight_channels(w, x.shape[-1])
        elif not transposed and x.shape[-1] % 8 != 0:
            ctx.cin_true = x.shape[-1]
            x, w = pad_input_channels(x, w)
        if _is_c1(w, ks, stride, transposed) and not want_stats:
            z, stats = conv3d_c1_forward(x, w.contiguous()), None
        elif transposed:
            Cout = w.shape[1]
            z, stats = deconv3d_forward(x, pack_weight(w, 2), Cout, want_stats=want_stats)
        else:
            Cout = w.shape[0]
            z, stats = conv3d_forward(x, pack_weight(w, 0), Cout, ks, stride, want_stats=want_stats)
        ctx.save_for_backward(x, w)
        ctx.cfg = (ks, stride, transposed)
        if stats is None:
            stats = x.new_empty(0)
        ctx.mark_non_differentiable(stats)
        return z, stats

    @staticmethod
    def backward(ctx, gz, _gstats):
        x, w = ctx.saved_tensors
        ks, stride, transposed = ctx.cfg
        pend = _take_pending_bn(gz)
        gx = gw = None
        B, D, H, W, Cin = x.shape
        if pend is not None:
            if (ctx.needs_input_grad[1] and not transposed and ks == 3 and stride == 1 and ctx.cin_true is None
                    and get_lib().raw("stx_conv3d_wgrad_bn_supported")(B, D, H, W, Cin, w.shape[0])):
                gw_pre, gz = conv3d_wgrad_bn(x, gz, pend)
                gw_pre = gw_pre.reshape(w.shape)
            else:
                gw_pre, gz = None, pend.materialize()
        else:
            gw_pre = None
        gz = gz.contiguous()
        if transposed:
            Ci, Co = w.shape[0], w.shape[1]
            if ctx.needs_input_grad[0]:
                gx, _ = conv3d_forward(gz, pack_weight(w, 0), Ci, 3, 2)
            if ctx.needs_input_grad[1]:
                gz_w = gz if Co % 32 == 0 else _pad_channels(gz, (Co + 31) // 32 * 32)
                x_w = x if Ci % 32 == 0 else _pad_channels(x, (Ci + 31) // 32 * 32)
                gw = conv3d_wgrad(gz_w, x_w, 3, 2)[:Ci, :Co].reshape(w.shape)
        else:
            Co, Ci = w.shape[0], w.shape[1]
            c1 = _is_c1(w, ks, stride, transposed)
            gz_k, w_k = gz, w
            if Co % 8 != 0 and not c1:
                Cp = (Co + 7) // 8 * 8
                gz_k = _pad_channels(gz, Cp)
                w_k = w.new_zeros(Cp, *w.shape[1:])
                w_k[:Co] = w
            if ctx.needs_input_grad[0]:
                if c1:
                    gx = conv3d_c1_dgrad(gz, w.contiguous(), Ci)
                elif stride == 1 and Ci > 128:
                    parts = []
                    for lo in range(0, Ci, 128):
                        hi = min(Ci, lo + 128)
                        g, _ = conv3d_forward(gz_k, pack_weight(w_k[:, lo:hi].contiguous(), 1), hi - lo, ks, 1)
                        parts.append(g)
                    gx = torch.cat(parts, -1)
                elif stride == 1:
                    gx, _ = conv3d_forward(gz_k, pack_weight(w_k, 1), Ci, ks, 1)
                else:
                    if Co % 32:
                        Cp = (Co + 31) // 32 * 32
                        gz_k = _pad_channels(gz, Cp)
                        w_k = w.new_zeros(Cp, *w.shape[1:])
                        w_k[:Co] = w
                    gx, _ = deconv3d_forward(gz_k, pack_weight(w_k, 2), Ci, out_dims=(D, H, W))
            if gw_pre is not None:
                gw = gw_pre
            elif ctx.needs_input_grad[1]:
                if c1:
                    gw = conv3d_c1_wgrad(x, gz)
                else:
                    gz_w = gz if Co % 32 == 0 else _pad_channels(gz, (Co + 31) // 32 * 32)
                    x_w = x if Ci % 32 == 0 else _pad_channels(x, (Ci + 31) // 32 * 32)
                    gw = conv3d_wgrad(x_w, gz_w, ks, stride)[:Co, :Ci].reshape(w.shape)
        if ctx.cin_true is not None:
            if gx is not None and not ctx.x_prepadded:
                gx = gx[..., :ctx.cin_true].contiguous()
            if gw is not None:
                gw = gw[:, :ctx.cin_true].contiguous()
        return gx, gw, None, None, None, None


class SharedInputConvsFn(torch.autograd.Function):

    @staticmethod
    def forward(ctx, x, cfgs, *ws):
        _chk(x, "x", 5)
        outs = []
        for (ks, stride, want), w in zip(cfgs, ws):
            if x.shape[-1] != w.shape[1] or w.shape[1] % 8 or w.shape[0] % 8 or _is_c1(w, ks, stride, False):
                raise StxError(f"SharedInputConvsFn: weight {tuple(w.shape)} on an input of {x.shape[-1]} channels")
            z, stats = conv3d_forward(x, pack_weight(w, 0), w.shape[0], ks, stride, want_stats=want)
            if stats is None:
                stats = x.new_empty(0)
            ctx.mark_non_differentiable(stats)
            outs += [z, stats]
        ctx.save_for_backward(x, *ws)
        ctx.cfgs = cfgs
        return tuple(outs)

    @staticmethod
    def backward(ctx, *grads):
        x, ws = ctx.saved_tensors[0], ctx.saved_tensors[1:]
        B, D, H, W, Ci = x.shape
        gws = [None] * len(ws)
        gzs = []
        for k, g in enumerate(grads[0::2]):
            pend = _take_pending_bn(g)
            if pend is not None:
                ks, stride, _ = ctx.cfgs[k]
                if (ctx.needs_input_grad[2 + k] and ks == 3 and stride == 1
                        and get_lib().raw("stx_conv3d_wgrad_bn_supported")(B, D, H, W, Ci, ws[k].shape[0])):
                    gw, g = conv3d_wgrad_bn(x, g, pend)
                    gws[k] = gw.reshape(ws[k].shape)
                else:
                    g = pend.materialize()
            gzs.append(None if g is None else g.contiguous())
        gx = None
        if ctx.needs_input_grad[0]:
            rank = lambda k: (0 if ctx.cfgs[k][0] == 3 and ctx.cfgs[k][1] == 1 else (1 if ctx.cfgs[k][1] == 2 else 2))
            for k in sorted((k for k in range(len(ws)) if gzs[k] is not None), key=rank):
                (ks, stride, _), w, gz = ctx.cfgs[k], ws[k], gzs[k]
                if stride == 1:
                    gx, _ = conv3d_forward(gz, pack_weight(w, 1), Ci, ks, 1, residual=gx)
                else:
                    Co = w.shape[0]
                    gz_k, w_k = gz, w
                    if Co % 32:
                        Cp = (Co + 31) // 32 * 32
                        gz_k = _pad_channels(gz, Cp)
                        w_k = w.new_zeros(Cp, *w.shape[1:])
                        w_k[:Co] = w
                    gx, _ = deconv3d_forward(gz_k, pack_weight(w_k, 2), Ci, out_dims=(D, H, W), residual=gx)
        for k, (w, gz) in enumerate(zip(ws, gzs)):
            if gz is None or not ctx.needs_input_grad[2 + k] or gws[k] is not None:
                continue
            ks, stride, _ = ctx.cfgs[k]
            Co = w.shape[0]
            gz_w = gz if Co % 32 == 0 else _pad_channels(gz, (Co + 31) // 32 * 32)
            x_w = x if Ci % 32 == 0 else _pad_channels(x, (Ci + 31) // 32 * 32)
            gws[k] = conv3d_wgrad(x_w, gz_w, ks, stride)[:Co, :Ci].reshape(w.shape)
        return (gx, None, *gws)


_D4_SEL = ((3, 1, 4), (4, 2, 0))


def embed_deconv4_weight(w):
    Ci, Co = w.shape[0], w.shape[1]
    wz = torch.cat((w, w.new_zeros(Ci, Co, 1, 4, 4)), 2)
    wz = torch.cat((wz, wz.new_zeros(Ci, Co, 5, 1, 4)), 3)
    wz = torch.cat((wz, wz.new_zeros(Ci, Co, 5, 5, 1)), 4)
    parts = []
    for pd in (0, 1):
        for ph in (0, 1):
            for pw in (0, 1):
                sel = wz[:, :, list(_D4_SEL[pd])][:, :, :, list(_D4_SEL[ph])][:, :, :, :, list(_D4_SEL[pw])]
                parts.append(sel.transpose(0, 1))
    return torch.cat(parts, 0).contiguous()


class DepthToSpaceFn(torch.autograd.Function):

    @staticmethod
    def forward(ctx, y):
        y = y.contiguous()
        _chk(y, "y", 5)
        B, D, H, W, C8 = y.shape
        C = C8 // 8
        out = torch.empty(B, 2 * D, 2 * H, 2 * W, C, dtype=torch.float32, device=y.device)
        _call("stx_depth_to_space", _p(y), _p(out), B, D, H, W, C, 0)
        return out

    @staticmethod
    def backward(ctx, g):
        g = g.contiguous()
        B, D2, H2, W2, C = g.shape
        gy = torch.empty(B, D2 // 2, H2 // 2, W2 // 2, 8 * C, dtype=torch.float32, device=g.device)
        _call("stx_depth_to_space", _p(g), _p(gy), B, D2 // 2, H2 // 2, W2 // 2, C, 1)
        return gy


def _d4_chunks(Co):
    per = max(1, min(8, 128 // Co))
    return [(c0, min(8, c0 + per)) for c0 in range(0, 8, per)]


def deconv4_raw(x, w, want_stats):
    Co = w.shape[1]
    if Co % 4:
        raise StxError(f"ConvTranspose3d(k4): {Co} output channels (need a multiple of 4)")
    w3 = embed_deconv4_weight(w)
    ys = [ConvRawFn.apply(x, w3[c0 * Co:c1 * Co], 3, 1, False, False)[0] for c0, c1 in _d4_chunks(Co)]
    z = DepthToSpaceFn.apply(ys[0] if len(ys) == 1 else torch.cat(ys, -1))
    return z, (bn_stats(z.detach()) if want_stats else z.new_empty(0))


@fp32_region
def deconv4_forward(x, w, scale=None, bias=None, relu=0, owner=None):
    _chk(x, "x", 5)
    Co = w.shape[1]
    if Co % 4:
        raise StxError(f"ConvTranspose3d(k4): {Co} output channels (need a multiple of 4)")
    cache = owner.__dict__.setdefault("_stx_packed", {}) if (owner is not None and _CACHE_ENABLED) else None
    key = (owner._version, owner.data_ptr()) if owner is not None else None
    hit = cache.get("d4") if cache is not None else None
    if hit is not None and hit[0] == key:
        packed = hit[1]
    else:
        w3 = embed_deconv4_weight(w)
        packed = [pack_weight(w3[c0 * Co:c1 * Co].contiguous(), 0) for c0, c1 in _d4_chunks(Co)]
        if cache is not None:
            cache["d4"] = (key, packed)
    ys = []
    for (c0, c1), wp in zip(_d4_chunks(Co), packed):
        n = c1 - c0
        ys.append(conv3d_forward(x, wp, n * Co, 3, 1, None if scale is None else scale.repeat(n),
                                 None if bias is None else bias.repeat(n), None, relu)[0])
    B, D, H, W, _ = x.shape
    y = ys[0] if len(ys) == 1 else torch.cat(ys, -1)
    out = torch.empty(B, 2 * D, 2 * H, 2 * W, Co, dtype=torch.float32, device=x.device)
    _call("stx_depth_to_space", _p(y), _p(out), B, D, H, W, Co, 0)
    return out


class GateFn(torch.autograd.Function):

    @staticmethod
    def forward(ctx, cv, att):
        out = gate(cv.detach(), att.detach())
        ctx.save_for_backward(cv, att)
        return out

    @staticmethod
    def backward(ctx, g):
        cv, att = ctx.saved_tensors
        g = g.contiguous()
        B, D, H, W, C = cv.shape
        gcv = torch.empty_like(cv) if ctx.needs_input_grad[0] else None
        gatt = torch.empty_like(att) if ctx.needs_input_grad[1] else None
        if gcv is not None or gatt is not None:
            _call("stx_gate_bwd", _p(g), _p(cv), _p(att), _p(gcv), _p(gatt), B, D, H * W, C)
        return gcv, gatt


@fp32_region
def gate(cv, att):
    if torch.is_grad_enabled() and (cv.requires_grad or att.requires_grad):
        return GateFn.apply(cv.contiguous(), att.contiguous())
    cv, att = cv.contiguous(), att.contiguous()
    _chk(cv, "cv", 5)
    _chk(att, "att", 4)
    B, D, H, W, C = cv.shape
    if att.shape != (B, H, W, C) or C % 4:
        raise StxError(f"gate: volume {tuple(cv.shape)} vs gate {tuple(att.shape)} (need [B,H,W,C], C % 4 == 0)")
    out = torch.empty_like(cv)
    _call("stx_gate_fwd", _p(cv), _p(att), _p(out), B, D, H * W, C)
    return out


class ChannelMajorFn(torch.autograd.Function):

    @staticmethod
    def forward(ctx, x):
        B, C, H, W = x.shape
        out = torch.empty((B, C, H, W), dtype=x.dtype, device=x.device)
        _call("stx_transpose", _p(x.permute(0, 2, 3, 1)), _p(out), B, H * W, C)
        return out

    @staticmethod
    def backward(ctx, g):
        g = g.contiguous()
        B, C, H, W = g.shape
        gx = torch.empty((B, H, W, C), dtype=g.dtype, device=g.device)
        _call("stx_transpose", _p(g), _p(gx), B, C, H * W)
        return gx.permute(0, 3, 1, 2)


@fp32_region
def channel_major(x):
    if x.is_contiguous():
        return x
    if (x.dim() == 4 and x.dtype == torch.float32 and on_device(x) and x.is_contiguous(memory_format=torch.channels_last)
            and x.shape[1] % 4 == 0 and (x.shape[2] * x.shape[3]) % 4 == 0):
        return ChannelMajorFn.apply(x)
    return x.contiguous()


class CatChannelsFn(torch.autograd.Function):

    @staticmethod
    def forward(ctx, *parts):
        ctx.cs = [int(p.shape[-1]) for p in parts]
        nvox = parts[0].numel() // ctx.cs[0]
        out = parts[0].new_empty(*parts[0].shape[:-1], sum(ctx.cs))
        ptrs = [_p(p) for p in parts] + [None] * (4 - len(parts))
        cs = ctx.cs + [0] * (4 - len(parts))
        _call("stx_concat_channels", *ptrs, *cs, _p(out), nvox)
        return out

    @staticmethod
    def backward(ctx, g):
        g = g.contiguous()
        nvox = g.numel() // g.shape[-1]
        outs = [g.new_empty(*g.shape[:-1], c) if need else None for c, need in zip(ctx.cs, ctx.needs_input_grad)]
        if any(o is not None for o in outs):
            dst = [o if o is not None else g.new_empty(*g.shape[:-1], c) for o, c in zip(outs, ctx.cs)]
            ptrs = [_p(o) for o in dst] + [None] * (4 - len(dst))
            cs = ctx.cs + [0] * (4 - len(dst))
            _call("stx_split_channels", _p(g), *ptrs, *cs, nvox)
        return tuple(outs)


@fp32_region
def cat_channels(parts):
    parts = [p.contiguous() for p in parts]
    if not 2 <= len(parts) <= 4:
        raise StxError(f"cat_channels: {len(parts)} parts (2 to 4)")
    lead = parts[0].shape[:-1]
    for p in parts:
        if p.shape[:-1] != lead or p.shape[-1] % 4 or p.dtype != torch.float32 or p.device != parts[0].device:
            raise StxError(f"cat_channels: parts {[tuple(q.shape) for q in parts]} (equal leading shape, fp32, widths % 4 == 0)")
    return CatChannelsFn.apply(*parts)


def conv2d_supported(conv):
    return (conv.kernel_size == (3, 3) and conv.stride == (1, 1) and conv.padding == (1, 1) and conv.dilation == (1, 1)
            and conv.groups == 1 and conv.bias is None and conv.in_channels in (32, 64) and conv.out_channels in (32, 64))


def _ohwi(w):
    v = w.permute(0, 2, 3, 1)
    return v if v.is_contiguous() else v.contiguous()


def conv2d_forward(x, w, dgrad=False, groups=1, want_stats=False):
    _chk(x, "x", 4)
    wo = _ohwi(w)
    _chk(wo, "weight", 4)
    B, H, W, Cin = x.shape
    Co, Ci = w.shape[0], w.shape[1]
    Kin, Nout = (Co, Ci) if dgrad else (Ci, Co)
    if Cin != Kin or B % groups:
        raise StxError(f"conv2d: input {tuple(x.shape)} against weight {tuple(w.shape)} (dgrad={dgrad}, groups={groups})")
    out = torch.empty(B, H, W, Nout, dtype=torch.float32, device=x.device)
    part = None
    if want_stats:
        rows = int(get_lib().raw("stx_conv2d_stat_rows")(groups))
        part = torch.empty(rows, 2, Nout, dtype=torch.float32, device=x.device)
    _call("stx_conv2d_fwd", _p(x), _p(wo), _p(out), _p(part), B, H, W, Kin, Nout, int(dgrad), groups)
    if part is not None and groups > 1:
        part = part.view(groups, rows // groups, 2, Nout)
    return out, part


class Conv2dFn(torch.autograd.Function):

    @staticmethod
    def forward(ctx, x, w, groups):
        xl = x.permute(0, 2, 3, 1)
        if not xl.is_contiguous():
            xl = xl.contiguous()
        z, part = conv2d_forward(xl, w, False, groups, True)
        ctx.save_for_backward(x, w)
        ctx.mark_non_differentiable(part)
        return z, part

    @staticmethod
    def backward(ctx, gz, _gpart):
        x, w = ctx.saved_tensors
        gz = gz.contiguous()
        gx = gw = None
        if ctx.needs_input_grad[0]:
            gx = conv2d_forward(gz, w, True)[0].permute(0, 3, 1, 2)
        if ctx.needs_input_grad[1]:
            gw = torch.ops.aten.convolution_backward(gz.permute(0, 3, 1, 2), x, w, None, (1, 1), (1, 1), (1, 1), False, (0, 0), 1,
                                                     (False, True, False))[1]
        return gx, gw, None


def bn_finalize(partials, count, gamma, beta, running_mean, running_var, momentum, eps, groups=1):
    C = partials.shape[-1]
    out = torch.empty(4, groups, C, dtype=torch.float32, device=partials.device)
    _call("stx_bn_finalize_groups", _p(partials), partials.shape[-3], C, float(count), _p(gamma), _p(beta),
          _p(running_mean), _p(running_var), float(momentum), float(eps), _p(out), groups)
    return list(out.unbind(0)) if groups > 1 else list(out[:, 0].unbind(0))


@fp32_region
def bn_stats(z, groups=1):
    _chk(z, "z")
    C = z.shape[-1]
    nvox = z.numel() // C // groups
    if groups < 1 or z.shape[0] % groups:
        raise StxError(f"bn_stats: leading axis {z.shape[0]} does not split into {groups} groups")
    rows = get_lib().raw("stx_bn_stats_rows")(nvox, C)
    if rows <= 0:
        raise StxError(f"bn_stats: C={C} unsupported")
    part = torch.empty(groups, rows, 2, C, dtype=torch.float32, device=z.device)
    _call("stx_bn_stats", _p(z), _p(part), nvox, C, groups)
    return part if groups > 1 else part[0]


def _sync_bn_partials(partials, count, group, world):
    import torch.distributed as dist
    tot = partials.double().sum(0)
    dist.all_reduce(tot, group=group)
    hi = tot.float()
    lo = (tot - hi.double()).float()
    return torch.stack((hi, lo)).contiguous(), count * world


@fp32_region
def bn_apply(z1, scale1, shift1, z2=None, scale2=None, shift2=None, relu=False, groups=1):
    out = torch.empty_like(z1)
    C = z1.shape[-1]
    _call("stx_bn_apply", _p(z1), _p(scale1), _p(shift1), _p(z2), _p(scale2), _p(shift2), _p(out),
          z1.numel() // C // groups, C, int(relu), groups)
    return out


class BnActFn(torch.autograd.Function):

    @staticmethod
    def forward(ctx, z1, gamma1, beta1, z2, gamma2, beta2, residual, relu, bn1, bn2, groups=1, defer=False):
        G = int(groups)
        ctx.defer = bool(defer)

        def affine(gamma, beta, bn):
            if bn["training"]:
                partials, count = bn["partials"], bn["count"]
                if bn.get("sync"):
                    if G > 1:
                        raise StxError("BnActFn: SyncBatchNorm with groups is not wired (SyncBN runs the views separately)")
                    partials, count = _sync_bn_partials(partials, count, *bn["sync"])
                return bn_finalize(partials, count, gamma, beta, bn["running_mean"], bn["running_var"], bn["momentum"],
                                   bn["eps"], G)
            invstd = torch.rsqrt(bn["running_var"] + bn["eps"])
            scale = gamma * invstd
            res = (scale, beta - bn["running_mean"] * scale, bn["running_mean"].clone(), invstd)
            return res if G == 1 else [t.unsqueeze(0).expand(G, -1).contiguous() for t in res]

        relu = int(relu)
        if relu == 2 and residual is not None:
            raise StxError("BnActFn: Mish with a plain residual is not wired (no model of the family uses it)")
        if G < 1 or z1.shape[0] % G:
            raise StxError(f"BnActFn: leading axis {z1.shape[0]} does not split into {G} groups")
        sc1, sh1, m1, i1 = affine(gamma1, beta1, bn1)
        two = z2 is not None
        if two:
            sc2, sh2, m2, i2 = affine(gamma2, beta2, bn2)
            y = bn_apply(z1, sc1, sh1, z2, sc2, sh2, relu, G)
        else:
            sc2 = sh2 = m2 = i2 = None
            y = bn_apply(z1, sc1, sh1, residual, None, None, relu, G)
        ctx.relu, ctx.two, ctx.has_res, ctx.groups = relu, two, residual is not None, G
        ctx.train1 = bn1["training"]
        ctx.train2 = bn2["training"] if two else False
        ctx.sync = bn1.get("sync") or (bn2.get("sync") if two else None)
        ctx.remask = bool(relu) and residual is None
        keep_y = y if (relu and not ctx.remask) else None
        ctx.save_for_backward(z1, gamma1, m1, i1, z2, gamma2, m2, i2, keep_y, sc1 if ctx.remask else None,
                              sh1 if ctx.remask else None, sc2 if (ctx.remask and two) else None,
                              sh2 if (ctx.remask and two) else None)
        return y

    @staticmethod
    def backward(ctx, gy):
        z1, gamma1, m1, i1, z2, gamma2, m2, i2, y, sc1, sh1, sc2, sh2 = ctx.saved_tensors
        gy = gy.contiguous()
        G = ctx.groups
        C = z1.shape[-1]
        nvox = z1.numel() // C // G
        lib = get_lib()
        NB = lib.raw("stx_bn_reduce_blocks")()
        part = _WS.get("bnred", G * NB * 3 * C, z1.device)
        sums_all = torch.empty(G + (1 if G > 1 else 0), 3, C, dtype=torch.float32, device=z1.device)
        sums = sums_all[:G]
        _call("stx_bn_bwd_reduce2", _p(gy), _p(y), _p(z1), _p(m1), _p(i1), _p(z2) if ctx.two else None,
              _p(m2) if ctx.two else None, _p(i2) if ctx.two else None, _p(sc1), _p(sh1), _p(sc2), _p(sh2), _p(part),
              _p(sums_all), nvox, C, int(ctx.relu), G)
        if not ctx.needs_input_grad[0] and not ctx.two and not ctx.has_res:
            tot = sums_all[G] if G > 1 else sums_all[0]
            return (None, tot[1], tot[0], None, None, None, None, None, None, None, None, None)
        if (ctx.defer and not ctx.two and not ctx.has_res and ctx.relu in (0, 1) and ctx.train1 and not ctx.sync and G == 1
                and (not ctx.relu or ctx.remask)):
            alias = gy.view_as(gy)
            pend = _PendingBn()
            pend.g, pend.z, pend.scale, pend.shift, pend.mean, pend.invstd = alias, z1, sc1, sh1, m1, i1
            pend.gamma, pend.sums, pend.inv_n, pend.act = gamma1, sums, 1.0 / nvox, int(ctx.relu)
            if pend.scale is None:
                pend.scale = pend.shift = m1
            _defer_pending_bn(alias, pend)
            tot = sums_all[0]
            return (alias, tot[1], tot[0], None, None, None, None, None, None, None, None, None)
        dz1 = torch.empty_like(z1)
        dz2 = torch.empty_like(z2) if ctx.two else None
        gres = torch.empty_like(z1) if (ctx.has_res and ctx.relu) else None
        use = sums
        if ctx.sync:
            import torch.distributed as dist
            use = sums.clone()
            dist.all_reduce(use, group=ctx.sync[0])
            use /= ctx.sync[1]
        if not ctx.train1 or (ctx.two and not ctx.train2):
            use = torch.zeros_like(sums)
        _call("stx_bn_bwd_apply2", _p(gy), _p(y), _p(z1), _p(m1), _p(i1), _p(gamma1), _p(z2) if ctx.two else None,
              _p(m2) if ctx.two else None, _p(i2) if ctx.two else None, _p(gamma2) if ctx.two else None, _p(sc1), _p(sh1),
              _p(sc2), _p(sh2), _p(use), _p(dz1), _p(dz2), _p(gres), nvox, C, int(ctx.relu), G)
        if ctx.has_res and not ctx.relu:
            gres = gy
        tot = sums_all[G] if G > 1 else sums_all[0]
        return (dz1, tot[1], tot[0], dz2, tot[2] if ctx.two else None, tot[0].clone() if ctx.two else None, gres,
                None, None, None, None, None)


class MishFn(torch.autograd.Function):

    @staticmethod
    def forward(ctx, x):
        x = x.contiguous()
        _chk(x, "x")
        y = torch.empty_like(x)
        _call("stx_mish_fwd", _p(x), _p(y), x.numel())
        ctx.save_for_backward(x)
        return y

    @staticmethod
    def backward(ctx, gy):
        (x,) = ctx.saved_tensors
        gy = gy.contiguous()
        gx = torch.empty_like(x)
        _call("stx_mish_bwd", _p(gy), _p(x), _p(gx), x.numel())
        return gx


@fp32_region
def mish(x):
    if torch.is_grad_enabled() and x.requires_grad:
        return MishFn.apply(x)
    x = x.contiguous()
    _chk(x, "x")
    y = torch.empty_like(x)
    _call("stx_mish_fwd", _p(x), _p(y), x.numel())
    return y


def _cv_shapes(Lg, Lc, num_groups):
    ref = Lg if Lg is not None else Lc
    B, _, H, W = ref.shape
    Cg = Lg.shape[1] if Lg is not None else 0
    Cc = Lc.shape[1] if Lc is not None else 0
    G = num_groups if Lg is not None else 0
    return B, H, W, Cg, G, Cc


@fp32_region
def cost_volume_forward(Lg, Rg, Lc, Rc, maxdisp, num_groups, mask_left=True, scale=None):
    for n, t in (("ref gwc", Lg), ("tgt gwc", Rg), ("ref concat", Lc), ("tgt concat", Rc)):
        _chk(t, n, 4)
    B, H, W, Cg, G, Cc = _cv_shapes(Lg, Lc, num_groups)
    if G:
        assert Cg % G == 0
    vol = torch.empty(B, maxdisp, H, W, G + 2 * Cc, dtype=torch.float32, device=(Lg if Lg is not None else Lc).device)
    _call("stx_cost_volume_fwd", _p(Lg), _p(Rg), Cg, G, _p(Lc), _p(Rc), Cc, _p(scale), _p(vol), B, H, W, maxdisp,
          int(mask_left))
    return vol


class CostVolumeFn(torch.autograd.Function):

    @staticmethod
    def forward(ctx, Lg, Rg, Lc, Rc, maxdisp, num_groups, mask_left):
        ctx.save_for_backward(Lg, Rg)
        ctx.cfg = (maxdisp, num_groups, mask_left, None if Lc is None else Lc.shape)
        return cost_volume_forward(Lg, Rg, Lc, Rc, maxdisp, num_groups, mask_left)

    @staticmethod
    def backward(ctx, gvol):
        Lg, Rg = ctx.saved_tensors
        maxdisp, num_groups, mask_left, cshape = ctx.cfg
        gvol = gvol.contiguous()
        B, D, H, W, CT = gvol.shape
        Cg = Lg.shape[1] if Lg is not None else 0
        G = num_groups if Lg is not None else 0
        Cc = cshape[1] if cshape is not None else 0
        gLg = torch.empty_like(Lg) if G else None
        gRg = torch.empty_like(Rg) if G else None
        gLc = gvol.new_empty(cshape) if Cc else None
        gRc = gvol.new_empty(cshape) if Cc else None
        _call("stx_cost_volume_bwd", _p(gvol), _p(Lg), _p(Rg), Cg, G, Cc, _p(gLg), _p(gRg), _p(gLc), _p(gRc), B, H, W,
              D, int(mask_left))
        return gLg, gRg, gLc, gRc, None, None, None


class GroupNormalizeFn(torch.autograd.Function):

    @staticmethod
    def forward(ctx, x, num_groups, out_scale):
        x = x.contiguous()
        _chk(x, "x", 4)
        B, C, H, W = x.shape
        y = torch.empty_like(x)
        _call("stx_group_normalize_fwd", _p(x), _p(y), B, C, num_groups, H * W, float(out_scale))
        ctx.save_for_backward(x)
        ctx.cfg = (num_groups, float(out_scale))
        return y

    @staticmethod
    def backward(ctx, gy):
        (x,) = ctx.saved_tensors
        gy = gy.contiguous()
        B, C, H, W = x.shape
        gx = torch.empty_like(x)
        _call("stx_group_normalize_bwd", _p(x), _p(gy), _p(gx), B, C, ctx.cfg[0], H * W, ctx.cfg[1])
        return gx, None, None


@fp32_region
def group_normalize(x, num_groups, out_scale=1.0):
    assert x.dim() == 4 and x.shape[1] % num_groups == 0, f"C:{x.shape[1]}, num_groups:{num_groups}"
    return GroupNormalizeFn.apply(channel_major(x), num_groups, out_scale)


@fp32_region
def cost_volume(Lg, Rg, Lc, Rc, maxdisp, num_groups, mask_left=True, normalize=False):
    if normalize and Lg is not None:
        Lg = group_normalize(Lg, num_groups, float(Lg.shape[1] // num_groups))
        Rg = group_normalize(Rg, num_groups, 1.0)
    ts = [channel_major(t) if t is not None else None for t in (Lg, Rg, Lc, Rc)]
    if torch.is_grad_enabled() and any(t is not None and t.requires_grad for t in ts):
        return CostVolumeFn.apply(*ts, maxdisp, num_groups, mask_left)
    return cost_volume_forward(*ts, maxdisp, num_groups, mask_left)


class SampledVolumeFn(torch.autograd.Function):

    @staticmethod
    def forward(ctx, Lg, Rg, Lc, Rc, samples, num_groups):
        B, H, W, Cg, G, Cc = _cv_shapes(Lg, Lc, num_groups)
        S = samples.shape[1]
        CTp = (G + 2 * Cc + 1 + 7) // 8 * 8
        vol = torch.empty(B, S, H, W, CTp, dtype=torch.float32, device=samples.device)
        _call("stx_sampled_volume_fwd", _p(Lg), _p(Rg), Cg, G, _p(Lc), _p(Rc), Cc, _p(samples), _p(vol), B, H, W, S, CTp)
        ctx.save_for_backward(Lg, Rg, samples)
        ctx.cfg = (G, Cg, Cc, None if Lc is None else Lc.shape)
        return vol

    @staticmethod
    def backward(ctx, gvol):
        Lg, Rg, samples = ctx.saved_tensors
        G, Cg, Cc, cshape = ctx.cfg
        gvol = gvol.contiguous()
        B, S, H, W, CTp = gvol.shape
        gLg = torch.empty_like(Lg) if G else None
        gRg = torch.empty_like(Rg) if G else None
        gLc = gvol.new_empty(cshape) if Cc else None
        gRc = gvol.new_empty(cshape) if Cc else None
        _call("stx_sampled_volume_bwd", _p(gvol), _p(Lg), _p(Rg), Cg, G, Cc, _p(samples), _p(gLg), _p(gRg), _p(gLc),
              _p(gRc), B, H, W, S, CTp)
        return gLg, gRg, gLc, gRc, None, None


@fp32_region
def sampled_volume(Lg, Rg, Lc, Rc, samples, num_groups):
    ts = [channel_major(t) if t is not None else None for t in (Lg, Rg, Lc, Rc)]
    for n, t in (("ref gwc", ts[0]), ("tgt gwc", ts[1]), ("ref concat", ts[2]), ("tgt concat", ts[3])):
        _chk(t, n, 4)
    samples = samples.detach().contiguous()
    _chk(samples, "samples", 4)
    if ts[0] is not None:
        assert ts[0].shape[1] % num_groups == 0
    if torch.is_grad_enabled() and any(t is not None and t.requires_grad for t in ts):
        return SampledVolumeFn.apply(*ts, samples, num_groups)
    return SampledVolumeFn.forward(_NoCtx(), *ts, samples, num_groups)


class _NoCtx:

    def save_for_backward(self, *a):
        pass
# ... 1383 lines not shown
```

Baseline: 0.1785 pairs/s.

## Fuse skip-gradient accumulation into conv dgrad and batch weight repacking

```diff
diff --git a/include/stx_hip.h b/include/stx_hip.h
--- a/include/stx_hip.h
+++ b/include/stx_hip.h
@@ -36,6 +36,8 @@
 
 long long stx_conv3d_packed_floats(int K, int N, int T);
 int stx_conv3d_pack_weight(const float* w, float* wp, int A, int B, int T, int mode, void* stream);
+int stx_conv3d_pack_multi_max_jobs(void);
+int stx_conv3d_pack_weights_multi(const float* const* ws, float* const* wps, const int* dims, int njobs, void* stream);
 int stx_conv3d_fwd_blocks(int Do, int Ho, int Wo);
 long long stx_conv3d_fwd_stat_rows(int B, int Di, int Hi, int Wi, int Cin, int Cout, int ks, int stride);
 int stx_conv3d_fwd(const float* x, const float* wp, float* out, const float* scale, const float* bias,
@@ -58,6 +60,8 @@
 long long stx_conv2d_stat_rows(int groups);
 int stx_conv2d_fwd(const float* x, const float* w, float* out, float* stats, int B, int H, int W, int Cin, int Cout, int dgrad,
                    int groups, void* stream);
+int stx_conv2d_dgrad_acc(const float* gz, const float* w, const float* acc, float* out, int B, int H, int W, int Cin, int Cout,
+                         void* stream);
 
 int stx_conv3d_c1_fwd(const float* x, const float* w, const float* residual, float* out, int B, int D, int H, int W,
                       int Cin, void* stream);
diff --git a/stereo_toolbox_amd/_capi.py b/stereo_toolbox_amd/_capi.py
--- a/stereo_toolbox_amd/_capi.py
+++ b/stereo_toolbox_amd/_capi.py
@@ -31,6 +31,8 @@
     "stx_split_mode": [_P, _P, _P, _I, _I, _I, _P],
     "stx_conv3d_packed_floats": [_I, _I, _I],
     "stx_conv3d_pack_weight": [_P, _P, _I, _I, _I, _I, _P],
+    "stx_conv3d_pack_multi_max_jobs": [],
+    "stx_conv3d_pack_weights_multi": [_P, _P, _P, _I, _P],
     "stx_conv3d_fwd_blocks": [_I, _I, _I],
     "stx_conv3d_fwd_stat_rows": [_I, _I, _I, _I, _I, _I, _I, _I],
     "stx_deconv3d_fwd_blocks": [_I, _I, _I],
@@ -43,6 +45,7 @@
     "stx_conv2d_supported": [_I, _I],
     "stx_conv2d_stat_rows": [_I],
     "stx_conv2d_fwd": [_P, _P, _P, _P, _I, _I, _I, _I, _I, _I, _I, _P],
+    "stx_conv2d_dgrad_acc": [_P, _P, _P, _P, _I, _I, _I, _I, _I, _P],
     "stx_conv3d_c1_fwd": [_P, _P, _P, _P, _I, _I, _I, _I, _I, _P],
     "stx_conv3d_c1_wgrad_workspace_floats": [_I],
     "stx_conv3d_c1_wgrad": [_P, _P, _P, _P, _I, _I, _I, _I, _I, _P],
diff --git a/stereo_toolbox_amd/aggregation.py b/stereo_toolbox_amd/aggregation.py
--- a/stereo_toolbox_amd/aggregation.py
+++ b/stereo_toolbox_amd/aggregation.py
@@ -159,6 +159,17 @@
 
 
 @ops.fp32_region
+def skip_input_conv(x, seq):
+    conv, bn = seq[0], seq[1]
+    if (_is_transposed(conv) or not bn.training or _conv_cfg(conv) != (3, 1) or conv.weight.shape[1] != x.shape[-1]
+            or conv.weight.shape[1] % 8 or conv.weight.shape[0] % 8 or conv.weight.shape[1] > 128
+            or not x.requires_grad or not _needs_grad(x) or os.environ.get("STX_SKIP_GRAD_ACC", "1") == "0"):
+        return None, x
+    z, part, res = ops.ConvSkipFn.apply(x, conv.weight, True)
+    return (z, part), res
+
+
+@ops.fp32_region
 def conv_block(x, conv, bn=None, relu=False, second=None, residual=None, mish=False, leaky=False, raw=None, second_raw=None):
     if (mish and relu) or (leaky and (relu or mish)):
         raise ops.StxError("conv_block: relu, mish and leaky are mutually exclusive")
diff --git a/stereo_toolbox_amd/csrc/conv2d.hip b/stereo_toolbox_amd/csrc/conv2d.hip
--- a/stereo_toolbox_amd/csrc/conv2d.hip
+++ b/stereo_toolbox_amd/csrc/conv2d.hip
@@ -10,6 +10,7 @@
     const float* w;
     float* out;
     float* stats;
+    const float* acc;
     int B, H, W, Cin, Cout;
     int nHt, nWt, groups;
     int dgrad;
@@ -17,7 +18,7 @@
 
 __device__ __forceinline__ f32x4 c2_zero4() { f32x4 z = {0.f, 0.f, 0.f, 0.f}; return z; }
 
-template <int KQ, int ABL = 0, int PAD = 8>
+template <int KQ, int ABL = 0, int PAD = 8, bool ACC = false>
 __global__ __launch_bounds__(C2_THREADS) void conv2d_march_kernel(Conv2dArgs a) {
     constexpr int CIN = 16 * KQ, VS = CIN + PAD, F4 = CIN / 4;
     constexpr int WFLOATS = 9 * KQ * 256;
@@ -102,6 +103,7 @@
     f32x4 pacc0 = c2_zero4(), pacc1 = c2_zero4();
     unsigned pvoff[2] = {STX_BUF_OOB, STX_BUF_OOB}, cvoff[2] = {STX_BUF_OOB, STX_BUF_OOB};
     stx_bufrsrc prs = stx_make_rsrc(a.out, 0u);
+    float4 pres[2] = {make_float4(0.f, 0.f, 0.f, 0.f), make_float4(0.f, 0.f, 0.f, 0.f)}, cres[2] = {pres[0], pres[0]};
     float s1[4] = {0.f, 0.f, 0.f, 0.f}, s2[4] = {0.f, 0.f, 0.f, 0.f};
     auto emit_prev = [&](int r) {
         f32x4 v = r ? pacc1 : pacc0;
@@ -112,6 +114,7 @@
             s1[c] += v[c];
             s2[c] = fmaf(v[c], v[c], s2[c]);
         }
+        if (ACC) { v[0] += pres[r].x; v[1] += pres[r].y; v[2] += pres[r].z; v[3] += pres[r].w; }
         stx_buf_st4(prs, pvoff[r], 0u, make_float4(v[0], v[1], v[2], v[3]));
     };
     auto flush_stats = [&](int slice) {
@@ -153,6 +156,7 @@
         const long long norg = (long long)(noh0 - 1) * a.W + (now0 - 1), img = (long long)a.H * a.W;
         const stx_bufrsrc nrs = stx_make_rsrc(a.x + ((long long)nb * img + norg) * CIN, more ? (unsigned)((img - norg) * CIN * 4) : 0u);
         const stx_bufrsrc crs = stx_make_rsrc(a.out + (size_t)b * img * a.Cout, (unsigned)(img * a.Cout * 4));
+        const stx_bufrsrc ars = stx_make_rsrc(ACC ? a.acc + (size_t)b * img * a.Cout : a.x, ACC ? (unsigned)(img * a.Cout * 4) : 0u);
         const float* pbuf = bufs + cur * SLOT;
         float* nbuf = bufs + (cur ^ 1) * SLOT;
         f32x4 acc0, acc1;
@@ -189,6 +193,7 @@
                 const int r = st - 8;
                 const int oh = oh0 + 2 * wave + r, ow = ow0 + i;
                 cvoff[r] = (unsigned)((((oh * a.W + ow) * a.Cout) + 16 * slice + 4 * kg) * 4) | (((oh < a.H) & (ow < a.W)) ? 0u : STX_BUF_OOB);
+                if (ACC) cres[r] = stx_buf_ld4(ars, cvoff[r], 0u);
             }
             if (st >= NSTEP - NST) {
                 const int k = st - (NSTEP - NST);
@@ -209,6 +214,7 @@
         prs = crs;
         pvoff[0] = cvoff[0]; pvoff[1] = cvoff[1];
         pacc0 = acc0; pacc1 = acc1;
+        if (ACC) { pres[0] = cres[0]; pres[1] = cres[1]; }
         if (!(ABL & 8)) __syncthreads();
         if (more && nslice != slice) {
             emit_prev(0); emit_prev(1);
@@ -248,16 +254,15 @@
     return groups >= 1 && groups <= 256 ? conv2d_grid(groups) : 0;
 }
 
-extern "C" int stx_conv2d_fwd(const float* x, const float* w, float* out, float* stats, int B, int H, int W, int Cin, int Cout,
-                              int dgrad, int groups, void* stream) {
-    stx_begin();
+static int conv2d_launch(const float* x, const float* w, float* out, float* stats, const float* acc, int B, int H, int W, int Cin,
+                         int Cout, int dgrad, int groups, void* stream) {
     STX_REQUIRE(x && w && out && B > 0 && H > 0 && W > 0 && (dgrad == 0 || dgrad == 1), "conv2d_fwd: bad args");
     STX_REQUIRE(stx_conv2d_supported(Cin, Cout), "conv2d_fwd: %d -> %d channels unsupported (Cin 32 or 64, Cout a multiple of 16)", Cin, Cout);
     STX_REQUIRE(groups >= 1 && groups <= 256 && B % groups == 0, "conv2d_fwd: batch %d does not split into %d groups", B, groups);
     STX_REQUIRE((long long)(H + 2) * W * (Cin > Cout ? Cin : Cout) * 4 < (1ll << 31), "conv2d_fwd: image too large for one descriptor");
     STX_REQUIRE(H < 32768 && W < 32768, "conv2d_fwd: image too large");
     Conv2dArgs a;
-    a.x = x; a.w = w; a.out = out; a.stats = stats; a.dgrad = dgrad;
+    a.x = x; a.w = w; a.out = out; a.stats = stats; a.acc = acc; a.dgrad = dgrad;
     a.B = B; a.H = H; a.W = W; a.Cin = Cin; a.Cout = Cout;
     a.nHt = stx_cdiv(H, C2_TH); a.nWt = stx_cdiv(W, C2_TW); a.groups = groups;
     const int grid = conv2d_grid(groups);
@@ -272,7 +277,24 @@
         k = abl == 1 ? conv2d_march_kernel<4, 1> : abl == 2 ? conv2d_march_kernel<4, 2> : abl == 3 ? conv2d_march_kernel<4, 3>
           : abl == 4 ? conv2d_march_kernel<4, 4> : abl == 7 ? conv2d_march_kernel<4, 7> : abl == 8 ? conv2d_march_kernel<4, 8>
           : conv2d_march_kernel<4, 15>;
+    if (acc) {
+        k = Cin == 64 ? conv2d_march_kernel<4, 0, 8, true> : conv2d_march_kernel<2, 0, 8, true>;
+        STX_REQUIRE(pad == 8, "conv2d_dgrad_acc: STX_C2_PAD is a profiling switch of conv2d_fwd");
+    }
     if (int rc = stx_lds_require((const void*)k, lds, "conv2d_fwd")) return rc;
     hipLaunchKernelGGL(k, dim3(grid), dim3(C2_THREADS), lds, (hipStream_t)stream, a);
     return stx_check_launch("conv2d_fwd");
 }
+
+extern "C" int stx_conv2d_fwd(const float* x, const float* w, float* out, float* stats, int B, int H, int W, int Cin, int Cout,
+                              int dgrad, int groups, void* stream) {
+    stx_begin();
+    return conv2d_launch(x, w, out, stats, nullptr, B, H, W, Cin, Cout, dgrad, groups, stream);
+}
+
+extern "C" int stx_conv2d_dgrad_acc(const float* gz, const float* w, const float* acc, float* out, int B, int H, int W, int Cin,
+                                    int Cout, void* stream) {
+    stx_begin();
+    STX_REQUIRE(acc && acc != out && ((uintptr_t)acc & 15) == 0, "conv2d_dgrad_acc: acc must be a 16-byte aligned tensor other than out");
+    return conv2d_launch(gz, w, out, nullptr, acc, B, H, W, Cin, Cout, 1, 1, stream);
+}
diff --git a/stereo_toolbox_amd/csrc/conv3d_pack.hip b/stereo_toolbox_amd/csrc/conv3d_pack.hip
--- /dev/null
+++ b/stereo_toolbox_amd/csrc/conv3d_pack.hip
@@ -0,0 +1,82 @@
+#include "stx_common.h"
+
+extern "C" long long stx_conv3d_packed_floats(int K, int N, int T);
+
+namespace {
+
+constexpr int PACK_THREADS = 256;
+constexpr int PACK_MAX_JOBS = 64;
+
+struct PackJob {
+    const float* w;
+    float* wp;
+    int A, Bd, T, mode;
+    unsigned blk0, total;
+};
+struct PackJobs {
+    PackJob job[PACK_MAX_JOBS];
+};
+
+__global__ __launch_bounds__(PACK_THREADS) void conv3d_pack_multi_kernel(PackJobs jobs, int njobs) {
+    PackJob jb = jobs.job[0];
+#pragma unroll
+    for (int t = 1; t < PACK_MAX_JOBS; ++t)
+        if (t < njobs && blockIdx.x >= jobs.job[t].blk0) jb = jobs.job[t];
+    const float* __restrict__ w = jb.w;
+    float* __restrict__ wp = jb.wp;
+    const int A = jb.A, Bd = jb.Bd, T = jb.T, mode = jb.mode;
+    const int K = (mode == 0) ? Bd : A, N = (mode == 0) ? A : Bd;
+    const int NT = N <= 32 ? 1 : (N <= 64 ? 2 : 4);
+    const size_t idx = (size_t)(blockIdx.x - jb.blk0) * PACK_THREADS + threadIdx.x;
+    if (idx >= jb.total) return;
+    const int j = idx & 3, lane = (idx >> 2) & 63;
+    size_t r = idx >> 8;
+    const int nt = r % NT; r /= NT;
+    const int NQ = K / 8;
+    const int q = r % NQ;
+    const int tap = r / NQ;
+    const int k = 8 * q + 4 * (lane >> 5) + j, n = 32 * nt + (lane & 31);
+    float v = 0.f;
+    if (n < N && k < K) {
+        if (mode == 0) v = w[((size_t)n * Bd + k) * T + tap];
+        else if (mode == 1) v = w[((size_t)k * Bd + n) * T + (T - 1 - tap)];
+        else v = w[((size_t)k * Bd + n) * T + tap];
+    }
+    wp[idx] = v;
+}
+
+}
+
+extern "C" int stx_conv3d_pack_multi_max_jobs() { return PACK_MAX_JOBS; }
+
+extern "C" int stx_conv3d_pack_weights_multi(const float* const* ws, float* const* wps, const int* dims, int njobs, void* stream) {
+    stx_begin();
+    const char* what = "conv3d_pack_weights_multi";
+    STX_REQUIRE(ws && wps && dims && njobs > 0, "%s: bad args", what);
+    for (int j = 0; j < njobs; ++j) {
+        const int A = dims[4 * j], Bd = dims[4 * j + 1], T = dims[4 * j + 2], mode = dims[4 * j + 3];
+        STX_REQUIRE(ws[j] && wps[j] && A > 0 && Bd > 0 && (T == 1 || T == 27), "%s: job %d: bad args", what, j);
+        STX_REQUIRE(mode >= 0 && mode <= 2, "%s: job %d: mode %d", what, j, mode);
+        const int K = (mode == 0) ? Bd : A, N = (mode == 0) ? A : Bd;
+        STX_REQUIRE(K % 8 == 0 && N <= 128, "%s: job %d: GEMM-K channels (%d) must be a multiple of 8, N (%d) <= 128", what, j, K, N);
+        STX_REQUIRE(stx_conv3d_packed_floats(K, N, T) < (1ll << 31), "%s: job %d: weight too large", what, j);
+    }
+    for (int j0 = 0; j0 < njobs; j0 += PACK_MAX_JOBS) {
+        const int n = njobs - j0 < PACK_MAX_JOBS ? njobs - j0 : PACK_MAX_JOBS;
+        PackJobs jobs = {};
+        unsigned blk = 0;
+        for (int t = 0; t < n; ++t) {
+            const int j = j0 + t;
+            PackJob& jb = jobs.job[t];
+            jb.w = ws[j]; jb.wp = wps[j];
+            jb.A = dims[4 * j]; jb.Bd = dims[4 * j + 1]; jb.T = dims[4 * j + 2]; jb.mode = dims[4 * j + 3];
+            const int K = (jb.mode == 0) ? jb.Bd : jb.A, N = (jb.mode == 0) ? jb.A : jb.Bd;
+            jb.total = (unsigned)stx_conv3d_packed_floats(K, N, jb.T);
+            jb.blk0 = blk;
+            blk += (jb.total + PACK_THREADS - 1) / PACK_THREADS;
+        }
+        hipLaunchKernelGGL(conv3d_pack_multi_kernel, dim3(blk), dim3(PACK_THREADS), 0, (hipStream_t)stream, jobs, n);
+        if (int rc = stx_check_launch(what)) return rc;
+    }
+    return STX_OK;
+}
diff --git a/stereo_toolbox_amd/models/ACVNet/acv.py b/stereo_toolbox_amd/models/ACVNet/acv.py
--- a/stereo_toolbox_amd/models/ACVNet/acv.py
+++ b/stereo_toolbox_amd/models/ACVNet/acv.py
@@ -2,7 +2,7 @@
 import torch.nn as nn
 
 from ... import ops
-from ...aggregation import convbn_block, deferred_bn_counters, shared_input_convs
+from ...aggregation import convbn_block, deferred_bn_counters, shared_input_convs, skip_input_conv
 from ..features2d import ResTrunk, cat_features, channels_last_weights_, convbn, init_reference_style, run_head2d, run_pair
 from ..GwcNet.gwcnet import classifier, run_classifier
 from .submodule import attention_block, convbn_3d
@@ -126,8 +126,9 @@
             ac = ops.ac_volume(cl, cr, prob, self.maxdisp // 4)
             cost0 = convbn_block(ac, self.dres0[0], relu=True)
             cost0 = convbn_block(cost0, self.dres0[2], relu=True)
-            t = convbn_block(cost0, self.dres1[0], relu=True)
-            cost0 = convbn_block(t, self.dres1[2], relu=False, residual=cost0)
+            raw, skip = skip_input_conv(cost0, self.dres1[0])
+            t = convbn_block(cost0, self.dres1[0], relu=True, raw=raw)
+            cost0 = convbn_block(t, self.dres1[2], relu=False, residual=skip)
             out1 = self.dres2(cost0)
             out2 = self.dres3(out1)
 
diff --git a/stereo_toolbox_amd/models/GwcNet/gwcnet.py b/stereo_toolbox_amd/models/GwcNet/gwcnet.py
--- a/stereo_toolbox_amd/models/GwcNet/gwcnet.py
+++ b/stereo_toolbox_amd/models/GwcNet/gwcnet.py
@@ -2,7 +2,7 @@
 import torch.nn as nn
 
 from ... import ops
-from ...aggregation import conv_block, convbn_block, deferred_bn_counters, shared_input_convs
+from ...aggregation import conv_block, convbn_block, deferred_bn_counters, shared_input_convs, skip_input_conv
 from ..features2d import ResTrunk, cat_features, channels_last_weights_, convbn, init_reference_style, run_head2d, run_pair
 from .submodule import convbn_3d
 
@@ -101,8 +101,9 @@
                               fr.get("concat_feature"), self.maxdisp // 4, self.num_groups, mask_left=True)
         cost0 = convbn_block(vol, self.dres0[0], relu=True)
         cost0 = convbn_block(cost0, self.dres0[2], relu=True)
-        t = convbn_block(cost0, self.dres1[0], relu=True)
-        cost0 = convbn_block(t, self.dres1[2], relu=False, residual=cost0)
+        raw, skip = skip_input_conv(cost0, self.dres1[0])
+        t = convbn_block(cost0, self.dres1[0], relu=True, raw=raw)
+        cost0 = convbn_block(t, self.dres1[2], relu=False, residual=skip)
         if self.training:
             out1, r0 = self.dres2(cost0, also=self.classif0[0])
             out2, r1 = self.dres3(out1, also=self.classif1[0])
diff --git a/stereo_toolbox_amd/models/PSMNet/stackhourglass.py b/stereo_toolbox_amd/models/PSMNet/stackhourglass.py
--- a/stereo_toolbox_amd/models/PSMNet/stackhourglass.py
+++ b/stereo_toolbox_amd/models/PSMNet/stackhourglass.py
@@ -1,7 +1,7 @@
 import torch.nn as nn
 
 from ... import ops
-from ...aggregation import conv_block, convbn_block, deferred_bn_counters
+from ...aggregation import conv_block, convbn_block, deferred_bn_counters, skip_input_conv
 from ..features2d import channels_last_weights_, init_reference_style, run_pair
 from .submodule import convbn_3d, feature_extraction
 
@@ -68,8 +68,9 @@
         cost = ops.cost_volume(None, None, fl, fr, self.maxdisp // 4, 0, mask_left=True)
         cost0 = convbn_block(cost, self.dres0[0], relu=True)
         cost0 = convbn_block(cost0, self.dres0[2], relu=True)
-        t = convbn_block(cost0, self.dres1[0], relu=True)
-        cost0 = convbn_block(t, self.dres1[2], relu=False, residual=cost0)
+        raw, skip = skip_input_conv(cost0, self.dres1[0])
+        t = convbn_block(cost0, self.dres1[0], relu=True, raw=raw)
+        cost0 = convbn_block(t, self.dres1[2], relu=False, residual=skip)
         out1, pre1, post1 = self.dres2(cost0, None, None, skip=cost0)
         out2, pre2, post2 = self.dres3(out1, pre1, post1, skip=cost0)
         out3, pre3, post3 = self.dres4(out2, pre1, post2, skip=cost0)
diff --git a/stereo_toolbox_amd/models/features2d.py b/stereo_toolbox_amd/models/features2d.py
--- a/stereo_toolbox_amd/models/features2d.py
+++ b/stereo_toolbox_amd/models/features2d.py
@@ -70,10 +70,18 @@
             and ops.conv2d_supported(conv) and x.shape[0] % view_groups.current() == 0)
 
 
-def conv_bn_act(x, conv, bn, relu=False, residual=None, second=None):
+def skip_grad_acc(x, conv, bn):
+    return (os.environ.get("STX_FEAT2D_SKIP_ACC", "1") != "0" and bn.training and own_conv2d(x, conv)
+            and torch.is_grad_enabled() and x.requires_grad)
+
+
+def conv_bn_act(x, conv, bn, relu=False, residual=None, second=None, skip=False):
     G = view_groups.current()
     part = None
-    if bn.training and own_conv2d(x, conv):
+    if skip:
+        zl, part, xs = ops.Conv2dFn.apply(x, conv.weight, G, True)
+        z = zl.permute(0, 3, 1, 2)
+    elif bn.training and own_conv2d(x, conv):
         zl, part = ops.Conv2dFn.apply(x, conv.weight, G)
         z = zl.permute(0, 3, 1, 2)
     else:
@@ -99,7 +107,7 @@
     else:
         y = ops.BnActFn.apply(zl, bn.weight, bn.bias, None, None, None, None if residual is None else _nhwc(residual),
                               relu, st, None, G)
-    return y.permute(0, 3, 1, 2)
+    return (y.permute(0, 3, 1, 2), xs) if skip else y.permute(0, 3, 1, 2)
 
 
 def convbn_relu_chain(seq, x):
@@ -145,6 +153,9 @@
     def forward(self, x):
         bns = [self.conv1[0][1], self.conv2[1]] + ([self.downsample[1]] if self.downsample is not None else [])
         if fused_glue(x, *bns):
+            if self.downsample is None and skip_grad_acc(x, self.conv1[0][0], self.conv1[0][1]):
+                y, xs = conv_bn_act(x, self.conv1[0][0], self.conv1[0][1], relu=True, skip=True)
+                return conv_bn_act(y, self.conv2[0], self.conv2[1], residual=xs)
             y = conv_bn_act(x, self.conv1[0][0], self.conv1[0][1], relu=True)
             if self.downsample is None:
                 return conv_bn_act(y, self.conv2[0], self.conv2[1], residual=x)
diff --git a/stereo_toolbox_amd/ops.py b/stereo_toolbox_amd/ops.py
--- a/stereo_toolbox_amd/ops.py
+++ b/stereo_toolbox_amd/ops.py
@@ -1,4 +1,7 @@
+import contextlib
 import ctypes
+import threading
+import weakref
 
 import torch
 
@@ -119,6 +122,8 @@
 def set_weight_cache(enabled):
     global _CACHE_ENABLED
     _CACHE_ENABLED = bool(enabled)
+    if not _CACHE_ENABLED:
+        _PACK_ARENA.clear()
 
 
 def invalidate_caches(model):
@@ -126,24 +131,103 @@
         m.__dict__.pop("_stx_fold", None)
     for p in model.parameters():
         p.__dict__.pop("_stx_packed", None)
-
-
-def pack_weight(w, mode, owner=None):
-    _chk(w, "weight", 5)
-    if owner is not None and _CACHE_ENABLED:
-        cache = owner.__dict__.setdefault("_stx_packed", {})
-        hit = cache.get(mode)
-        if hit is not None and hit[0] == (owner._version, owner.data_ptr()):
-            return hit[1]
+    _PACK_ARENA.forget(model.parameters())
+
+
+class _PackEntry:
+    __slots__ = ("ref", "key", "wp", "dims", "shape", "served")
+
+
+class _PackArena:
+
+    def __init__(self):
+        self.plans = {}
+        self.lock = threading.RLock()
+
+    def plan(self, device):
+        key = (device.index, torch.cuda.current_stream(device).cuda_stream if device.type == "cuda" else 0)
+        return self.plans.setdefault(key, {})
+
+    def size(self):
+        with self.lock:
+            return sum(len(p) for p in self.plans.values())
+
+    def clear(self):
+        with self.lock:
+            self.plans.clear()
+
+    def forget(self, tensors):
+        ids = {id(t) for t in tensors}
+        with self.lock:
+            for plan in self.plans.values():
+                for k in [k for k in plan if k[0] in ids]:
+                    del plan[k]
+
+    def record(self, plan, src, mode, wp, dims):
+        e = _PackEntry()
+        k = (id(src), mode)
+
+        def dead(_ref, plan=plan, k=k, lock=self.lock):
+            with lock:
+                if plan.get(k) is not None and plan[k].ref is _ref:
+                    del plan[k]
+        e.ref, e.key, e.wp, e.dims, e.shape = weakref.ref(src, dead), (src._version, src.data_ptr()), wp, dims, tuple(src.shape)
+        e.served = False
+        plan[k] = e
+        return e
+
+    def refresh(self, plan, device):
+        live, jobs = [], []
+        for k, e in list(plan.items()):
+            t = e.ref()
+            if t is None or t.device != device or tuple(t.shape) != e.shape or t.dtype != torch.float32 or not t.is_contiguous():
+                plan.pop(k, None)
+                continue
+            live.append(t)
+            jobs.append((e, (t._version, t.data_ptr())))
+        if not jobs:
+            return
+        n = len(jobs)
+        ws = (ctypes.c_void_p * n)(*[key[1] for _, key in jobs])
+        wps = (ctypes.c_void_p * n)(*[e.wp.data_ptr() for e, _ in jobs])
+        dims = (ctypes.c_int * (4 * n))(*[d for e, _ in jobs for d in e.dims])
+        with torch.cuda.device(device) if device.type == "cuda" else contextlib.nullcontext():
+            _call("stx_conv3d_pack_weights_multi", ws, wps, dims, n)
+        for e, key in jobs:
+            e.key, e.served = key, False
+
+
+_PACK_ARENA = _PackArena()
+
+
+def _pack_single(w, mode):
     A, Bd = w.shape[0], w.shape[1]
     T = w.shape[2] * w.shape[3] * w.shape[4]
     K, N = (Bd, A) if mode == 0 else (A, Bd)
     n = get_lib().raw("stx_conv3d_packed_floats")(K, N, T)
     wp = torch.empty(n, dtype=torch.float32, device=w.device)
     _call("stx_conv3d_pack_weight", _p(w), _p(wp), A, Bd, T, mode)
-    if owner is not None and _CACHE_ENABLED:
-        cache[mode] = ((owner._version, owner.data_ptr()), wp)
-    return wp
+    return wp, (A, Bd, T, mode)
+
+
+def pack_weight(w, mode, owner=None):
+    _chk(w, "weight", 5)
+    src = w if owner is None else owner
+    if (not _CACHE_ENABLED or (w.is_cuda and torch.cuda.is_current_stream_capturing())
+            or (src is not w and (src.data_ptr() != w.data_ptr() or src.shape != w.shape))):
+        return _pack_single(w, mode)[0]
+    with _PACK_ARENA.lock:
+        plan = _PACK_ARENA.plan(w.device)
+        e = plan.get((id(src), mode))
+        if e is not None and e.ref() is src and (e.key != (src._version, src.data_ptr()) or (owner is None and e.served)):
+            _PACK_ARENA.refresh(plan, w.device)
+            e = plan.get((id(src), mode))
+        if e is None or e.ref() is not src or e.key != (src._version, src.data_ptr()):
+            wp, dims = _pack_single(w, mode)
+            e = _PACK_ARENA.record(plan, src, mode, wp, dims)
+        if owner is None:
+            e.served = True
+        return e.wp
 
 
 def _pad_channels(t, C):
@@ -480,6 +564,46 @@
         return (gx, None, *gws)
 
 
+class ConvSkipFn(torch.autograd.Function):
+
+    @staticmethod
+    def forward(ctx, x, w, want_stats):
+        _chk(x, "x", 5)
+        Co, Ci = w.shape[0], w.shape[1]
+        if x.shape[-1] != Ci or Ci % 8 or Co % 8 or Ci > 128 or tuple(w.shape[2:]) != (3, 3, 3) or _is_c1(w, 3, 1, False):
+            raise StxError(f"ConvSkipFn: weight {tuple(w.shape)} on an input of {x.shape[-1]} channels")
+        z, stats = conv3d_forward(x, pack_weight(w, 0), Co, 3, 1, want_stats=want_stats)
+        ctx.save_for_backward(x, w)
+        if stats is None:
+            stats = x.new_empty(0)
+        ctx.mark_non_differentiable(stats)
+        return z, stats, x.view_as(x)
+
+    @staticmethod
+    def backward(ctx, gz, _gstats, gskip):
+        x, w = ctx.saved_tensors
+        B, D, H, W, Ci = x.shape
+        Co = w.shape[0]
+        gx = gw = None
+        pend = _take_pending_bn(gz)
+        if pend is not None:
+            if ctx.needs_input_grad[1] and get_lib().raw("stx_conv3d_wgrad_bn_supported")(B, D, H, W, Ci, Co):
+                gw, gz = conv3d_wgrad_bn(x, gz, pend)
+                gw = gw.reshape(w.shape)
+            else:
+                gz = pend.materialize()
+        if gz is None:
+            return gskip, None, None
+        gz = gz.contiguous()
+        if ctx.needs_input_grad[0]:
+            gx, _ = conv3d_forward(gz, pack_weight(w, 1), Ci, 3, 1, residual=None if gskip is None else gskip.contiguous())
+        if gw is None and ctx.needs_input_grad[1]:
+            gz_w = gz if Co % 32 == 0 else _pad_channels(gz, (Co + 31) // 32 * 32)
+            x_w = x if Ci % 32 == 0 else _pad_channels(x, (Ci + 31) // 32 * 32)
+            gw = conv3d_wgrad(x_w, gz_w, 3, 1)[:Co, :Ci].reshape(w.shape)
+        return gx, gw, None
+
+
 _D4_SEL = ((3, 1, 4), (4, 2, 0))
 
 
@@ -691,29 +815,48 @@
     return out, part
 
 
+def conv2d_dgrad_acc(gz, w, acc):
+    _chk(gz, "gz", 4)
+    _chk(acc, "acc", 4)
+    wo = _ohwi(w)
+    _chk(wo, "weight", 4)
+    B, H, W, Cin = gz.shape
+    Co, Ci = w.shape[0], w.shape[1]
+    if Cin != Co or tuple(acc.shape) != (B, H, W, Ci):
+        raise StxError(f"conv2d_dgrad_acc: gradient {tuple(gz.shape)} and acc {tuple(acc.shape)} against weight {tuple(w.shape)}")
+    out = torch.empty(B, H, W, Ci, dtype=torch.float32, device=gz.device)
+    _call("stx_conv2d_dgrad_acc", _p(gz), _p(wo), _p(acc), _p(out), B, H, W, Co, Ci)
+    return out
+
+
 class Conv2dFn(torch.autograd.Function):
 
     @staticmethod
-    def forward(ctx, x, w, groups):
+    def forward(ctx, x, w, groups, skip=False):
         xl = x.permute(0, 2, 3, 1)
         if not xl.is_contiguous():
             xl = xl.contiguous()
         z, part = conv2d_forward(xl, w, False, groups, True)
         ctx.save_for_backward(x, w)
         ctx.mark_non_differentiable(part)
-        return z, part
-
-    @staticmethod
-    def backward(ctx, gz, _gpart):
+        return (z, part, x.view_as(x)) if skip else (z, part)
+
+    @staticmethod
+    def backward(ctx, gz, _gpart, gskip=None):
         x, w = ctx.saved_tensors
+        if gz is None:
+            return (gskip, None, None, None)[:len(ctx.needs_input_grad)]
         gz = gz.contiguous()
         gx = gw = None
-        if ctx.needs_input_grad[0]:
+        if ctx.needs_input_grad[0] and gskip is not None:
+            acc = gskip.permute(0, 2, 3, 1)
+            gx = conv2d_dgrad_acc(gz, w, acc if acc.is_contiguous() else acc.contiguous()).permute(0, 3, 1, 2)
+        elif ctx.needs_input_grad[0]:
             gx = conv2d_forward(gz, w, True)[0].permute(0, 3, 1, 2)
         if ctx.needs_input_grad[1]:
             gw = torch.ops.aten.convolution_backward(gz.permute(0, 3, 1, 2), x, w, None, (1, 1), (1, 1), (1, 1), False, (0, 0), 1,
                                                      (False, True, False))[1]
-        return gx, gw, None
+        return (gx, gw, None, None)[:len(ctx.needs_input_grad)]
 
 
 def bn_finalize(partials, count, gamma, beta, running_mean, running_var, momentum, eps, groups=1):
```

Result: no change. 0.1783 pairs/s (-0.1%).
